# ForJadeForest/DistillCLIP

Hardware: AMD Instinct MI355X
Metric: image-text pairs/sec (distill step) (higher is better)
Workload: dtype bf16; 1 GPU; l_clip.yaml dual distill: ViT-B/32 CLIP teacher -> weight-shared ViT(6x768,24h,R2) + text(4x768,12h,R2) students, 224px/77tok, losses out_l1+out_cos+0.1*cos_diff, fwd+loss+bwd+AdamW; global_batch=512, batch_per_gpu=512, parallelism=dp1, gradient_exchange=none, negatives=local (reference training_step semantics), optimizer_in_step=True, teacher_residual=fp16, saved_gelu_derivative=u8 fixed point, clock_probe=True

## Files before the change

distillclip_amd/csrc/encoder.cpp:

```cpp
#include <math.h>
#include <stdlib.h>
#include <string.h>
#include <new>
#include <vector>
#include "common.h"

namespace {

#define CK(expr)                      \
    do {                              \
        int _rc = (expr);             \
        if (_rc != DCLIP_OK) return _rc; \
    } while (0)

enum { P_PER_TBLOCK = 12, P_PER_SBLOCK = 8, P_PER_SREPEAT = 6 };

struct Plan {
    dclip_encoder_cfg c;
    int D, H, hd, N, Np, F, E, L, R;
    int K;
    int Kp;
    bool student, image, compressed;
    bool mixing;
    bool train;
    struct EmbP { int table, w, bias, cls, pos, ln_w, ln_b; } emb;
    int p_blocks;
    struct HeadP { int norm_w, norm_b, head_w, head_b; } head;
    int n_params;
    struct BlockW { int64_t qkv, qkv_t, proj, proj_t, fc1, fc1_t, fc2, fc2_t; };
    std::vector<BlockW> bw;
    int64_t w_embed, w_embed_t, w_head, w_head_t, w_total;
};

int64_t wtake(int64_t& off, int64_t n) { int64_t o = off; off += (n + 127) & ~(int64_t)127; return o; }

bool make_plan(const dclip_encoder_cfg& c, Plan& p) {
    p.c = c;
    p.student = c.kind == 1; p.train = c.kind != 0; p.image = c.modality == 0; p.mixing = p.student && c.head_mix;
    p.D = c.width; p.H = c.heads; p.N = c.tokens; p.F = c.mlp_dim; p.E = c.out_dim; p.L = c.layers; p.R = c.repeats;
    if (c.kind < 0 || c.kind > 2 || c.modality < 0 || c.modality > 1) { dclip_set_error("encoder: bad kind/modality"); return false; }
    if (p.D <= 0 || p.H <= 0 || p.D % p.H) { dclip_set_error("encoder: width %d not divisible by heads %d", p.D, p.H); return false; }
    p.hd = p.D / p.H;
    if (p.hd != 32 && p.hd != 64) { dclip_set_error("encoder: head dim %d unsupported (32 or 64)", p.hd); return false; }
    if (p.D % 64 || p.F % 64 || p.E % 64 || p.D > 1024) { dclip_set_error("encoder: width/mlp/out dims must be multiples of 64, width <= 1024"); return false; }
    const bool long_ok = c.kind == 0 && p.image && !c.causal && p.hd == 64;
    if (p.N <= 0 || p.N > (long_ok ? 640 : 128)) {
        if (long_ok) dclip_set_error("encoder: tokens must be in 1..640 for a frozen image tower (got %d)", p.N);
        else if (p.N > 128 && c.kind != 0) dclip_set_error("encoder: tokens must be in 1..128 for a trainable tower (kind %d; got %d): only frozen image towers run longer sequences", c.kind, p.N);
        else if (p.N > 128 && !p.image) dclip_set_error("encoder: tokens must be in 1..128 for a text tower (got %d): only frozen image towers run longer sequences", p.N);
        else if (p.N > 128) dclip_set_error("encoder: tokens must be in 1..128 for a causal or head-dim-%d tower (got %d): longer sequences need a non-causal tower with head dim 64", p.hd, p.N);
        else dclip_set_error("encoder: tokens must be in 1..128 (got %d)", p.N);
        return false;
    }
    if (p.L <= 0 || p.R <= 0 || (!p.student && p.R != 1)) { dclip_set_error("encoder: bad layers/repeats"); return false; }
    p.Np = (p.N + 7) & ~7;
    p.compressed = !p.image && c.embed_rank > 0;
    p.K = p.Kp = 0;
    if (p.image) {
        if (c.patch <= 0 || c.resolution < c.patch || c.in_chans <= 0) { dclip_set_error("encoder: bad patch geometry"); return false; }
        const int g = c.resolution / c.patch;
        if (g * g + 1 != p.N) { dclip_set_error("encoder: tokens %d != (res/patch)^2 + 1 = %d", p.N, g * g + 1); return false; }
        p.K = c.in_chans * c.patch * c.patch;
        p.Kp = p.K;
        if (p.K % 64) {
            if (p.train) { dclip_set_error("encoder: in_chans*patch^2 = %d must be a multiple of 64 in a trainable tower", p.K); return false; }
            if (c.patch % 2) { dclip_set_error("encoder: patch %d must be even", c.patch); return false; }
            p.Kp = (p.K + 63) & ~63;
        }
    } else {
        if (c.vocab <= 0) { dclip_set_error("encoder: vocab required for text"); return false; }
        if (p.compressed && c.embed_rank % 64) { dclip_set_error("encoder: embed_rank must be a multiple of 64"); return false; }
        if (p.compressed && !p.student) { dclip_set_error("encoder: a compressed token embedding exists for the weight-shared student only (kind 1)"); return false; }
        if (p.compressed) p.K = p.Kp = c.embed_rank;
    }
    if (p.mixing && p.H != 2 && p.H != 4 && p.H != 8 && p.H != 12 && p.H != 24) {
        dclip_set_error("encoder: head count %d unsupported by the head-mixing kernels", p.H); return false;
    }
    int n = 0;
    Plan::EmbP& em = p.emb;
    em = Plan::EmbP{-1, -1, -1, -1, -1, -1, -1};
    if (p.image) {
        em.w = n++;
        if (p.student) em.bias = n++;
        em.cls = n++; em.pos = n++;
        if (!p.student) { em.ln_w = n++; em.ln_b = n++; }
    } else {
        em.table = n++;
        if (p.compressed) { em.w = n++; em.bias = n++; }
        em.pos = n++;
    }
    p.p_blocks = n;
    n += p.student ? p.L * (P_PER_SBLOCK + p.R * P_PER_SREPEAT) : p.L * P_PER_TBLOCK;
    p.head.norm_w = n++; p.head.norm_b = n++; p.head.head_w = n++;
    p.head.head_b = p.student ? n++ : -1;
    p.n_params = n;
    int64_t off = 0;
    const int64_t D = p.D, F = p.F, E = p.E;
    p.bw.resize(p.L);
    for (int l = 0; l < p.L; ++l) {
        auto& b = p.bw[l];
        b.qkv = wtake(off, 3 * D * D); b.proj = wtake(off, D * D); b.fc1 = wtake(off, F * D); b.fc2 = wtake(off, D * F);
        if (p.train) { b.qkv_t = wtake(off, 3 * D * D); b.proj_t = wtake(off, D * D); b.fc1_t = wtake(off, F * D); b.fc2_t = wtake(off, D * F); }
        else b.qkv_t = b.proj_t = b.fc1_t = b.fc2_t = -1;
    }
    p.w_embed = p.w_embed_t = -1;
    if (em.w >= 0) p.w_embed = wtake(off, D * p.Kp);
    if (p.compressed) p.w_embed_t = wtake(off, D * p.K);
    p.w_head = wtake(off, E * D);
    p.w_head_t = p.train ? wtake(off, E * D) : -1;
    p.w_total = off;
    return true;
}

enum class AttnPath { Fused, Mix, Unfused };
inline AttnPath attn_path(const Plan& p, bool training) {
    static const int mode = [] { const char* e = getenv("DCLIP_ATTN_MIX"); return e ? atoi(e) : 1; }();
    if (!training && !p.mixing) return AttnPath::Fused;
    if (p.mixing && mode != 0 && !p.c.causal && dclip_attn_mix_supported(p.H, p.N, p.hd) != 0) return AttnPath::Mix;
    return AttnPath::Unfused;
}

struct ExecSave {
    void* x_mid;
    float* mean1; float* rstd1; float* mean2; float* rstd2;
    bf16_t *h1, *qkv, *ctx, *h2, *u;
    uint8_t* z;
    float* S;
    bf16_t* P;
    bf16_t* Rm;
    float* stats;
};

void take_scores(Bump& b, const Plan& p, AttnPath path, int64_t B, int64_t N, int64_t Np, ExecSave& s) {
    const int64_t SN = B * p.H * N * Np;
    const bool unfused = path == AttnPath::Unfused;
    s.S = unfused ? b.take<float>(SN) : nullptr;
    s.P = unfused ? b.take<bf16_t>(SN) : nullptr;
    s.Rm = p.mixing ? b.take<bf16_t>(SN) : s.P;
    s.stats = path == AttnPath::Mix ? b.take<float>(B * p.H * N) : nullptr;
}

struct RowSet {
    bf16_t* ctx;
    void *xin, *x_mid, *xout;
    bf16_t *h2, *u;
    float *mean2, *rstd2; uint8_t* z;
    int64_t rows;
};

struct Work {
    std::vector<void*> X;
    bool h16;
    std::vector<ExecSave> ex;
    bf16_t* patches;
    float* tok_table;
    int32_t* pick;
    float *meanf, *rstdf;
    bf16_t* hf;
    void* x0;
    float *mean0, *rstd0;
    float* G0;
    float* G; bf16_t* Gb;
    bf16_t *gb_f2, *gb_pr;
    bf16_t *dbig, *dh, *dqkv, *dout;
    bf16_t* dR;
    bf16_t* dS;
    float* tok_sum; float* demb;
    float* wg_dummy;
    float* mix_ws; size_t mix_ws_bytes;
    void* tn_ws; size_t tn_ws_bytes;
    RowSet compact;
    bf16_t* ctx_full;
    float* Gc;
    AttnPath path;
    size_t bytes;
};

void layout(const Plan& p, int64_t B, bool training, void* base, Work& w, int64_t N = 0) {
    Bump b(base);
    w = Work{};
    if (N <= 0) N = p.N;
    const int64_t Npad = (N + 7) & ~(int64_t)7;
    const int64_t M = B * N, D = p.D, F = p.F, SN = B * p.H * N * Npad;
    const int nex = p.L * p.R;
    const bool save = p.train && training;
    w.path = attn_path(p, save);
    const bool mix = w.path == AttnPath::Mix, unfused = w.path == AttnPath::Unfused;
    w.X.assign(nex + 1, nullptr);
    w.ex.assign(nex, ExecSave{});
    ExecSave shared{};
    void* xs = nullptr;
    w.h16 = !p.train;
    if (!save) {
        xs = w.h16 ? (void*)b.take<_Float16>(M * D) : (void*)b.take<float>(M * D);
        shared.x_mid = xs;
        shared.h1 = b.take<bf16_t>(M * D); shared.qkv = b.take<bf16_t>(M * 3 * D);
        take_scores(b, p, w.path, B, N, Npad, shared);
        shared.ctx = b.take<bf16_t>(M * D); shared.h2 = shared.h1; shared.u = b.take<bf16_t>(M * F);
    }
    for (int e = 0; e <= nex; ++e) w.X[e] = save ? (void*)b.take<float>(M * D) : xs;
    for (int e = 0; e < nex; ++e) {
        if (!save) { w.ex[e] = shared; continue; }
        ExecSave& s = w.ex[e];
        s.x_mid = b.take<float>(M * D);
        s.mean1 = b.take<float>(M); s.rstd1 = b.take<float>(M); s.mean2 = b.take<float>(M); s.rstd2 = b.take<float>(M);
        s.qkv = b.take<bf16_t>(M * 3 * D);
        take_scores(b, p, w.path, B, N, Npad, s);
        s.z = b.take<uint8_t>(M * F);
        if (e % p.R == 0) {
            bf16_t* h1 = b.take<bf16_t>(p.R * M * D); bf16_t* ctx = b.take<bf16_t>(p.R * M * D);
            bf16_t* h2 = b.take<bf16_t>(p.R * M * D); bf16_t* u = b.take<bf16_t>(p.R * M * F);
            for (int r = 0; r < p.R; ++r) {
                ExecSave& t = w.ex[e + r];
                t.h1 = h1 + r * M * D; t.ctx = ctx + r * M * D; t.h2 = h2 + r * M * D; t.u = u + r * M * F;
            }
        }
    }
    {
        const ExecSave& s = w.ex[nex - 1];
        if (save) {
            w.ctx_full = s.h2;
            w.compact = RowSet{s.ctx, w.X[nex], s.x_mid, w.X[nex], s.h2, s.u, s.mean2, s.rstd2, s.z, B};
        } else {
            w.ctx_full = shared.ctx;
            bf16_t* cctx = b.take<bf16_t>(B * D);
            const size_t es = w.h16 ? 2 : 4;
            void* xr = b.take<char>(B * D * es); void* xmc = b.take<char>(B * D * es); void* xoc = b.take<char>(B * D * es);
            w.compact = RowSet{cctx, xr, xmc, xoc, shared.h1, shared.u, nullptr, nullptr, nullptr, B};
        }
        w.Gc = save ? b.take<float>(B * D) : nullptr;
    }
    w.patches = p.emb.w >= 0 ? b.take<bf16_t>(M * p.Kp) : nullptr;
    w.tok_table = b.take<float>((int64_t)N * D);
    w.pick = b.take<int32_t>(B);
    w.meanf = b.take<float>(B); w.rstdf = b.take<float>(B);
    w.hf = b.take<bf16_t>(B * D);
    const bool pre_ln = p.emb.ln_w >= 0, pre = save && pre_ln;
    w.x0 = pre_ln ? (w.h16 ? (void*)b.take<_Float16>(M * D) : (void*)b.take<float>(M * D)) : nullptr;
    w.mean0 = pre ? b.take<float>(M) : nullptr; w.rstd0 = pre ? b.take<float>(M) : nullptr; w.G0 = pre ? b.take<float>(M * D) : nullptr;
    if (save) {
        w.G = b.take<float>(M * D); w.Gb = b.take<bf16_t>(M * D);
        w.gb_f2 = b.take<bf16_t>(p.R * M * D); w.gb_pr = b.take<bf16_t>(p.R * M * D);
        w.dbig = b.take<bf16_t>(p.R * M * F); w.dh = b.take<bf16_t>(M * D); w.dqkv = b.take<bf16_t>(p.R * M * 3 * D);
        w.dR = unfused ? b.take<bf16_t>(SN) : nullptr; w.dS = b.take<bf16_t>(SN); w.dout = b.take<bf16_t>(B * p.E);
        w.tok_sum = b.take<float>((int64_t)N * D);
        w.wg_dummy = mix ? b.take<float>(2 * p.H * p.H) : nullptr;
        w.mix_ws_bytes = mix ? dclip_attn_mix_bwd_workspace_bytes(B, p.H, N) : 0;
        w.mix_ws = w.mix_ws_bytes ? (float*)b.take<char>(w.mix_ws_bytes) : nullptr;
        w.tn_ws_bytes = dclip_gemm_tn_workspace_bytes();
        w.tn_ws = b.take<char>(w.tn_ws_bytes);
        w.demb = p.compressed ? b.take<float>(M * p.K) : nullptr;
    }
    w.bytes = b.off;
}

inline RowSet full_rows(const Work& w, int ei, int64_t M) {
    const ExecSave& s = w.ex[ei];
    return RowSet{s.ctx, w.X[ei], s.x_mid, w.X[ei + 1], s.h2, s.u, s.mean2, s.rstd2, s.z, M};
}

inline const float* PF(const void* const* params, int i) { return i < 0 ? nullptr : (const float*)params[i]; }

inline int wsplits(int64_t M, int64_t P, int64_t Q) {
    const double tiles = (double)((P + 127) / 128) * (double)((Q + 127) / 128);
    const int smax = (int)((M + 255) / 256);
    int best = 1;
    double best_t = 1e30;
    for (int s = 1; s <= smax && s <= 64; ++s) {
        const double blocks = tiles * s;
        const double rounds = ceil(blocks / 512.0);
        const double t_mm = rounds * (2.0 * 128 * 128 * ((double)M / s)) / 1.76e12;
        const double t_at = 0.5 * s * (double)P * Q * 4.0 / 1.3e12;
        const double t = t_mm + t_at + 2e-6;
        if (t < best_t) { best_t = t; best = s; }
    }
    return best;
}

inline int gemm(const void* A, int64_t lda, const void* Bw, int64_t ldb, void* C, int64_t ldc, int64_t M, int64_t N, int64_t K,
                const float* bias, int act, const void* aux_in, void* aux_out, const void* res, int64_t ldr, int out_dtype,
                int64_t row_group, const float* rowadd, void* st) {
    return dclip_gemm_nt(A, lda, Bw, ldb, C, ldc, M, N, K, 1.f, bias, act, aux_in, aux_out, res, ldr, out_dtype, row_group, rowadd, nullptr, st);
}

inline int ln_stream(bool h16, const void* x, int64_t ldx, const int32_t* ridx, const float* g, const float* b, void* y, int64_t ldy, int out_dtype,
                     float* mean, float* rstd, int64_t M, int64_t D, void* st) {
    if (h16) return dclip_layernorm_fwd_f16(x, ldx, ridx, g, b, y, ldy, out_dtype, mean, rstd, M, D, 1e-5f, st);
    return dclip_layernorm_fwd((const float*)x, ldx, ridx, g, b, y, ldy, out_dtype, mean, rstd, M, D, 1e-5f, st);
}

inline int export_stream(bool h16, const void* src, float* dst, int64_t n, void* st) {
    if (h16) return dclip_cast_f16_f32(src, dst, n, st);
    if (hipMemcpyAsync(dst, src, (size_t)n * 4, hipMemcpyDeviceToDevice, (hipStream_t)st) != hipSuccess) {
        dclip_set_error("dclip_encoder_forward: hidden-state export failed");
        return DCLIP_ELAUNCH;
    }
    return DCLIP_OK;
}

int attn_forward(AttnPath path, const Plan& p, const ExecSave& s, const float* wl, const float* ww, int64_t B, int64_t N, const int32_t* pick,
                 void* st) {
    const int64_t D = p.D, H = p.H, hd = p.hd, Np = (N + 7) & ~(int64_t)7;
    const float scale = 1.f / sqrtf((float)hd);
    if (path == AttnPath::Fused) {
        if (N <= 128 && pick) return dclip_attn_fused_fwd_rows(s.qkv, 3 * D, s.ctx, D, B, H, N, hd, scale, p.c.causal, pick, st);
        if (N <= 128) return dclip_attn_fused_fwd(s.qkv, 3 * D, s.ctx, D, B, H, N, hd, scale, p.c.causal, st);
        return dclip_attn_stream_fwd(s.qkv, 3 * D, s.ctx, D, B, H, N, hd, scale, st);
    }
    const int blk = path == AttnPath::Mix ? 1 : 0;
    if (path == AttnPath::Mix) {
        if (pick) CK(dclip_attn_mix_fwd_rows(s.qkv, 3 * D, wl, ww, s.Rm, s.stats, B, H, N, Np, hd, scale, pick, st));
        else CK(dclip_attn_mix_fwd(s.qkv, 3 * D, wl, ww, s.Rm, s.stats, B, H, N, Np, hd, scale, st));
    } else {
        CK(dclip_attn_nt(s.qkv, 3 * D, s.qkv + D, 3 * D, s.S, 1, B, H, N, Np, hd, scale, st));
        CK(dclip_attn_softmax_fwd(s.S, wl, ww, wl ? s.P : nullptr, s.Rm, B, H, N, Np, p.c.causal, st));
    }
    if (pick) return dclip_attn_nn_rows(s.Rm, s.qkv + 2 * D, 3 * D, s.ctx, D, B, H, N, Np, hd, 1.f, blk, pick, 0, st);
    return dclip_attn_nn(s.Rm, s.qkv + 2 * D, 3 * D, s.ctx, D, B, H, N, Np, hd, 1.f, blk, st);
}

struct MapGrad { const float* d_score; const float* d_prob; void* scratch; size_t scratch_bytes; };
int attn_backward(AttnPath path, const Plan& p, const ExecSave& s, const Work& w, const float* wl, const float* ww, float* gl, float* gw,
                  const bf16_t* dctx, bf16_t* dqkv, int64_t B, const MapGrad* mg, const int32_t* pick, void* st) {
    const int64_t D = p.D, H = p.H, hd = p.hd, N = p.N, Np = p.Np;
    const float scale = 1.f / sqrtf((float)hd);
    const int blk = path == AttnPath::Mix ? 1 : 0;
    if (pick) {
        CK(dclip_attn_tn_rows(s.Rm, dctx, D, dqkv + 2 * D, 3 * D, B, H, N, Np, hd, 1.f, blk, pick, st));
        if (path == AttnPath::Mix) {
            CK(dclip_attn_mix_bwd_rows(s.qkv, 3 * D, dctx, D, wl, ww, s.stats, w.dS, gl ? gl : w.wg_dummy, gw ? gw : w.wg_dummy + H * H,
                                       w.mix_ws, w.mix_ws_bytes, B, H, N, Np, hd, scale, pick, st));
        } else {
            CK(dclip_attn_nt(dctx, D, s.qkv + 2 * D, 3 * D, w.dR, 0, B, H, N, Np, hd, 1.f, st));
            CK(dclip_attn_softmax_bwd(w.dR, s.P, s.S, 0, wl, ww, w.dS, gl, gw, B, H, N, Np, st));
        }
        CK(dclip_attn_nn_rows(w.dS, s.qkv + D, 3 * D, dqkv, 3 * D, B, H, N, Np, hd, scale, blk, pick, 1, st));
        return dclip_attn_tn_rows(w.dS, s.qkv, 3 * D, dqkv + D, 3 * D, B, H, N, Np, hd, scale, blk, pick, st);
    }
    CK(dclip_attn_tn(s.Rm, dctx, D, dqkv + 2 * D, 3 * D, B, H, N, Np, hd, 1.f, blk, st));
    if (path == AttnPath::Mix) {
        CK(dclip_attn_mix_bwd(s.qkv, 3 * D, dctx, D, wl, ww, s.stats, w.dS, gl ? gl : w.wg_dummy, gw ? gw : w.wg_dummy + H * H,
                              w.mix_ws, w.mix_ws_bytes, B, H, N, Np, hd, scale, st));
    } else {
        CK(dclip_attn_nt(dctx, D, s.qkv + 2 * D, 3 * D, w.dR, 0, B, H, N, Np, hd, 1.f, st));
        CK(dclip_attn_softmax_bwd(w.dR, s.P, s.S, 0, wl, ww, w.dS, gl, gw, B, H, N, Np, st));
    }
    if (mg) CK(dclip_attn_maps_bwd(s.qkv, 3 * D, wl, mg->d_score, mg->d_prob, w.dS, blk, gl, mg->scratch, mg->scratch_bytes, B, H, N, Np, hd,
                                   scale, p.c.causal, st));
    CK(dclip_attn_nn(w.dS, s.qkv + D, 3 * D, dqkv, 3 * D, B, H, N, Np, hd, scale, blk, st));
    return dclip_attn_tn(w.dS, s.qkv, 3 * D, dqkv + D, 3 * D, B, H, N, Np, hd, scale, blk, st);
}

}

enum : uint32_t { RUN_SEEDS_CLEAR = 1u, RUN_PRUNED = 2u, RUN_PRUNED_ATTN = 4u };

struct dclip_encoder { Plan p; };

extern "C" dclip_encoder* dclip_encoder_create(const dclip_encoder_cfg* cfg) {
    if (!cfg) { dclip_set_error("dclip_encoder_create: null cfg"); return nullptr; }
    dclip_encoder* e = new (std::nothrow) dclip_encoder();
    if (!e) { dclip_set_error("dclip_encoder_create: out of host memory"); return nullptr; }
    if (!make_plan(*cfg, e->p)) { delete e; return nullptr; }
    return e;
}

extern "C" void dclip_encoder_destroy(dclip_encoder* e) { delete e; }
extern "C" int64_t dclip_encoder_num_params(const dclip_encoder* e) { return e ? e->p.n_params : -1; }
extern "C" size_t dclip_encoder_wcache_bytes(const dclip_encoder* e) { return e ? dclip_up256((size_t)e->p.w_total * 2) : 0; }

extern "C" size_t dclip_encoder_workspace_bytes(const dclip_encoder* e, int64_t B, int training) {
    if (!e || B <= 0) return 0;
    Work w;
    layout(e->p, B, training != 0, nullptr, w);
    return w.bytes;
}

namespace {
struct BX { int n1w, n1b, n2w, n2b, qkvw, qkvb, prw, prb, f1w, f1b, f2w, f2b, cl, cw; };
inline BX bexec(const Plan& p, int l, int r) {
    if (!p.student) {
        const int b = p.p_blocks + l * P_PER_TBLOCK;
        return BX{b, b + 1, b + 6, b + 7, b + 2, b + 3, b + 4, b + 5, b + 8, b + 9, b + 10, b + 11, -1, -1};
    }
    const int b = p.p_blocks + l * (P_PER_SBLOCK + p.R * P_PER_SREPEAT), q = b + P_PER_SBLOCK + r * P_PER_SREPEAT;
    return BX{q, q + 1, q + 2, q + 3, b, b + 1, b + 2, b + 3, b + 4, b + 5, b + 6, b + 7, q + 4, q + 5};
}

struct EP { const float *n1w, *n1b, *n2w, *n2b, *bq, *bp, *b1, *b2, *wl, *ww; };
inline EP exec_params(const Plan& p, const void* const* params, int l, int r) {
    const BX bx = bexec(p, l, r);
    EP e{PF(params, bx.n1w), PF(params, bx.n1b), PF(params, bx.n2w), PF(params, bx.n2b), PF(params, bx.qkvb), PF(params, bx.prb),
         PF(params, bx.f1b), PF(params, bx.f2b), nullptr, nullptr};
    if (p.mixing) { e.wl = PF(params, bx.cl); e.ww = PF(params, bx.cw); }
    return e;
}

int exec_attn(const Plan& p, AttnPath path, const ExecSave& s, const bf16_t* W, int l, const EP& e, bool h16, const void* xin, int64_t B,
              int64_t N, const int32_t* pick, void* st) {
    const int64_t D = p.D, M = B * N;
    CK(ln_stream(h16, xin, D, nullptr, e.n1w, e.n1b, s.h1, D, DCLIP_OUT_BF16, s.mean1, s.rstd1, M, D, st));
    CK(gemm(s.h1, D, W + p.bw[l].qkv, D, s.qkv, 3 * D, M, 3 * D, D, e.bq, 0, nullptr, nullptr, nullptr, 0, DCLIP_OUT_BF16, 0, nullptr, st));
    return attn_forward(path, p, s, e.wl, e.ww, B, N, pick, st);
}

int exec_mlp(const Plan& p, const bf16_t* W, int l, const EP& e, bool h16, const RowSet& rs, void* st) {
    const int64_t D = p.D, F = p.F, rows = rs.rows;
    const auto& bw = p.bw[l];
    const int sdt = h16 ? DCLIP_OUT_F16 : DCLIP_OUT_F32;
    const int act = p.student ? (rs.z ? DCLIP_ACT_GELU_SAVE : DCLIP_ACT_GELU) : (rs.z ? DCLIP_ACT_QUICKGELU_SAVE : DCLIP_ACT_QUICKGELU);
    CK(gemm(rs.ctx, D, W + bw.proj, D, rs.x_mid, D, rows, D, D, e.bp, 0, nullptr, nullptr, rs.xin, D, sdt, 0, nullptr, st));
    CK(ln_stream(h16, rs.x_mid, D, nullptr, e.n2w, e.n2b, rs.h2, D, DCLIP_OUT_BF16, rs.mean2, rs.rstd2, rows, D, st));
    CK(gemm(rs.h2, D, W + bw.fc1, D, rs.u, F, rows, F, D, e.b1, act, nullptr, rs.z, nullptr, 0, DCLIP_OUT_BF16, 0, nullptr, st));
    return gemm(rs.u, F, W + bw.fc2, F, rs.xout, D, rows, D, F, e.b2, 0, nullptr, nullptr, rs.x_mid, D, sdt, 0, nullptr, st);
}

size_t llo_scratch(const Plan& p, AttnPath path, bool h16, int64_t B, void* base, void* xin, ExecSave& t, RowSet& rs) {
    Bump b(base);
    const int64_t N = p.N, M = B * N, D = p.D, F = p.F;
    const size_t es = h16 ? 2 : 4;
    t = ExecSave{};
    t.h1 = b.take<bf16_t>(M * D); t.h2 = t.h1;
    t.qkv = b.take<bf16_t>(M * 3 * D);
    take_scores(b, p, path, B, N, p.Np, t);
    t.ctx = b.take<bf16_t>(M * D);
    t.x_mid = b.take<char>(M * D * es);
    t.u = b.take<bf16_t>(M * F);
    rs = RowSet{t.ctx, xin, t.x_mid, b.take<char>(M * D * es), t.h2, t.u, nullptr, nullptr, nullptr, M};
    return b.off;
}

inline bool prune_last_enabled() {
    static const int v = [] { const char* e = getenv("DCLIP_PRUNE_LAST"); return e ? atoi(e) : 1; }();
    return v != 0;
}
inline bool prune_attn_enabled() {
    static const int v = [] { const char* e = getenv("DCLIP_PRUNE_ATTN"); return e ? atoi(e) : 1; }();
    return v != 0;
}

template <class T> struct ExecMaps { std::vector<T*> score, prob; uint64_t score_bits = 0, prob_bits = 0; };
template <class T>
int exec_maps(const Plan& p, const dclip_attn_maps* maps, T* const* score, T* const* prob, const dclip_encoder_run* rec, const char* fn,
              ExecMaps<T>& out) {
    const int nex = p.L * p.R;
    out.score.assign(nex, nullptr); out.prob.assign(nex, nullptr);
    if (!maps || !maps->n) return DCLIP_OK;
    DCLIP_REQUIRE(maps->n > 0 && maps->exec, "%s: maps need n > 0 execution indices", fn);
    for (int k = 0; k < maps->n; ++k) {
        const int ei = maps->exec[k];
        DCLIP_REQUIRE(ei >= 0 && ei < nex, "%s: map %d: block execution %d out of range 0..%d", fn, k, ei, nex - 1);
        T* sm = score ? score[k] : nullptr;
        T* pm = prob ? prob[k] : nullptr;
        if (!rec) {
            DCLIP_REQUIRE(ei < 64, "%s: map %d: block execution %d: maps are exported for executions 0..63 only", fn, k, ei);
        } else {
            const bool had_s = ei < 64 && (rec->score_maps >> ei & 1), had_p = ei < 64 && (rec->prob_maps >> ei & 1);
            DCLIP_REQUIRE((!sm || had_s) && (!pm || had_p), "%s: a gradient for the %s map of block execution %d, which the forward did not export",
                          fn, sm && !had_s ? "score" : "probability", ei);
        }
        if (sm) { out.score[ei] = sm; out.score_bits |= (uint64_t)1 << ei; }
        if (pm) { out.prob[ei] = pm; out.prob_bits |= (uint64_t)1 << ei; }
    }
    return DCLIP_OK;
}
}

extern "C" int dclip_encoder_prepare(const dclip_encoder* e, const void* const* params, void* wcache, void* st) {
    DCLIP_REQUIRE(e && params && wcache, "dclip_encoder_prepare: null argument");
    const Plan& p = e->p;
    bf16_t* W = (bf16_t*)wcache;
    const int64_t D = p.D, F = p.F, E = p.E;
    auto at = [&](int64_t off) -> void* { return off < 0 ? nullptr : (void*)(W + off); };
    std::vector<const float*> src; std::vector<void*> wb, wt; std::vector<int64_t> rr, cc;
    auto job = [&](const float* w, void* b, void* t, int64_t R, int64_t C) { src.push_back(w); wb.push_back(b); wt.push_back(t); rr.push_back(R); cc.push_back(C); };
    for (int l = 0; l < p.L; ++l) {
        const auto& b = p.bw[l];
        const BX bx = bexec(p, l, 0);
        job(PF(params, bx.qkvw), at(b.qkv), at(b.qkv_t), 3 * D, D);
        job(PF(params, bx.prw), at(b.proj), at(b.proj_t), D, D);
        job(PF(params, bx.f1w), at(b.fc1), at(b.fc1_t), F, D);
        job(PF(params, bx.f2w), at(b.fc2), at(b.fc2_t), D, F);
    }
    const bool pad_embed = p.Kp != p.K;
    if (p.emb.w >= 0 && !pad_embed) job(PF(params, p.emb.w), at(p.w_embed), at(p.w_embed_t), D, p.K);
    if (p.student) job(PF(params, p.head.head_w), at(p.w_head), at(p.w_head_t), E, D);
    else job(PF(params, p.head.head_w), at(p.w_head_t), at(p.w_head), D, E);
    for (size_t i = 0; i < src.size(); ++i) DCLIP_REQUIRE(src[i], "dclip_encoder_prepare: parameter %zu missing", i);
    if (pad_embed) {
        DCLIP_REQUIRE(PF(params, p.emb.w), "dclip_encoder_prepare: the patch-embedding weight is missing");
        CK(dclip_cast_bf16_pad(PF(params, p.emb.w), at(p.w_embed), D, p.K, p.Kp, st));
    }
    return dclip_cast_transpose_bf16_multi(src.data(), wb.data(), wt.data(), rr.data(), cc.data(), (int64_t)src.size(), st);
}

static int clear_backward_seeds(const Plan& p, const Work& w, int64_t M, int64_t B, bool pruned, void* st) {
    const int64_t D = p.D;
    hipStream_t hs = (hipStream_t)st;
    bf16_t* gb_last = w.gb_f2 + (int64_t)(p.R - 1) * M * D;
    const bool ok = pruned ? hipMemsetAsync(w.Gc, 0, (size_t)B * D * 4, hs) == hipSuccess
                           : hipMemsetAsync(w.G, 0, (size_t)M * D * 4, hs) == hipSuccess && hipMemsetAsync(gb_last, 0, (size_t)M * D * 2, hs) == hipSuccess;
    if (!ok) { dclip_set_error("dclip_encoder: clearing the backward seeds failed"); return DCLIP_ELAUNCH; }
    return DCLIP_OK;
}

extern "C" int dclip_encoder_forward(const dclip_encoder* e, const void* input, const void* patches, int64_t B, const void* const* params,
                                     const void* wcache, void* workspace, size_t ws_bytes, dclip_encoder_run* run, int training,
                                     float* last_representation, float* const* rep_out, float* emb_out, int64_t tokens_eff,
                                     const dclip_attn_maps* maps, void* st) {
    DCLIP_REQUIRE(e && (input || patches) && params && wcache && workspace && run && last_representation, "dclip_encoder_forward: null argument");
    DCLIP_REQUIRE(B > 0, "dclip_encoder_forward: empty batch");
    const Plan& p = e->p;
    const bf16_t* ext_patches = (const bf16_t*)patches;
    DCLIP_REQUIRE(!ext_patches || (p.image && ((uintptr_t)ext_patches % 16) == 0), "dclip_encoder_forward: patches: image towers only, 16-byte aligned rows");
    DCLIP_REQUIRE(!ext_patches || tokens_eff == 0, "dclip_encoder_forward: patches cannot be combined with tokens_eff");
    DCLIP_REQUIRE(!ext_patches || p.Kp == p.K, "dclip_encoder_forward: this tower pads its patch rows (%d -> %d columns) and cuts them itself: pass the images", p.K, p.Kp);
    DCLIP_REQUIRE(!training || p.train, "dclip_encoder_forward: the frozen teacher tower (kind 0) is inference-only");
    DCLIP_REQUIRE(tokens_eff == 0 || (!p.train && !p.image && p.c.causal && tokens_eff > 0 && tokens_eff <= p.N && !rep_out && !emb_out),
                  "dclip_encoder_forward: tokens_eff is only valid for the causal text teacher without hidden-state export");
    DCLIP_REQUIRE(!(maps && maps->n > 0 && maps->exec) || tokens_eff == 0,
                  "dclip_encoder_forward: attention maps cannot be exported from a caption prefix (tokens_eff)");
    DCLIP_REQUIRE(!(maps && maps->n > 0) || p.N <= 128,
                  "dclip_encoder_forward: attention maps cannot be exported from a tower of %d tokens (dclip_attn_maps_fwd / _bwd take N <= 128)", p.N);
    ExecMaps<float> xm;
    CK(exec_maps<float>(p, maps, maps ? maps->score : nullptr, maps ? maps->prob : nullptr, nullptr, "dclip_encoder_forward", xm));
    Work w;
    layout(p, B, training != 0, workspace, w, tokens_eff);
    DCLIP_REQUIRE(ws_bytes >= w.bytes, "dclip_encoder_forward: workspace too small (%zu < %zu)", ws_bytes, w.bytes);
    DCLIP_REQUIRE(((uintptr_t)workspace % 256) == 0 && ((uintptr_t)wcache % 256) == 0, "dclip_encoder_forward: buffers must be 256-byte aligned");
    const bf16_t* W = (const bf16_t*)wcache;
    const int64_t N = tokens_eff ? tokens_eff : p.N, D = p.D, F = p.F, E = p.E, M = B * N;
    const int nex = p.L * p.R;

    const Plan::EmbP& em = p.emb;
    const bool pre_ln = em.ln_w >= 0;
    const int sdt = w.h16 ? DCLIP_OUT_F16 : DCLIP_OUT_F32;
    if (em.w >= 0) {
        const bf16_t* rows = ext_patches ? ext_patches : w.patches;
        if (!p.image) CK(dclip_embed_gather((const int64_t*)input, p.N, PF(params, em.table), nullptr, w.patches, 0, M, N, p.K, st));
        else if (!ext_patches && p.Kp != p.K) CK(dclip_im2row_ld((const float*)input, w.patches, p.Kp, B, p.c.in_chans, p.c.resolution, p.c.patch, 1, st));
        else if (!ext_patches) CK(dclip_im2row((const float*)input, w.patches, B, p.c.in_chans, p.c.resolution, p.c.patch, 1, st));
        CK(dclip_token_table(PF(params, em.pos), PF(params, em.cls), PF(params, em.bias), w.tok_table, N, D, st));
        CK(gemm(rows, p.Kp, W + p.w_embed, p.Kp, pre_ln ? w.x0 : w.X[0], D, M, D, p.Kp, nullptr, 0, nullptr, nullptr, nullptr, 0, sdt, N, w.tok_table, st));
        if (pre_ln) CK(ln_stream(w.h16, w.x0, D, nullptr, PF(params, em.ln_w), PF(params, em.ln_b), w.X[0], D, sdt, w.mean0, w.rstd0, M, D, st));
    } else {
        CK(dclip_embed_gather((const int64_t*)input, p.N, PF(params, em.table), PF(params, em.pos), w.X[0], sdt, M, N, D, st));
    }

    if (emb_out) CK(export_stream(w.h16, pre_ln ? w.x0 : w.X[0], emb_out, M * D, st));

    CK(dclip_pick_index(p.image ? nullptr : (const int64_t*)input, p.N, w.pick, B, N, st));
    const bool prune = prune_last_enabled() && !(rep_out && rep_out[nex - 1]) && !xm.score[nex - 1] && !xm.prob[nex - 1];
    const bool prune_attn = prune && prune_attn_enabled() && N <= 128;
    for (int ei = 0; ei < nex; ++ei) {
        const int l = ei / p.R, r = ei % p.R;
        const ExecSave& s = w.ex[ei];
        const EP ep = exec_params(p, params, l, r);
        const bool compact = prune && ei == nex - 1;
        ExecSave sa = s;
        if (compact) sa.ctx = w.ctx_full;
        CK(exec_attn(p, w.path, sa, W, l, ep, w.h16, w.X[ei], B, N, compact && prune_attn ? w.pick : nullptr, st));
        if (xm.score[ei] || xm.prob[ei]) CK(dclip_attn_maps_fwd(s.qkv, 3 * D, ep.wl, xm.score[ei], xm.prob[ei], B, p.H, N, p.hd, 1.f / sqrtf((float)p.hd), p.c.causal, st));
        if (compact) {
            CK(dclip_rows_pick(w.ctx_full, w.compact.ctx, w.pick, B, D * 2, st));
            CK(dclip_rows_pick(w.X[ei], w.compact.xin, w.pick, B, D * (w.h16 ? 2 : 4), st));
        }
        CK(exec_mlp(p, W, l, ep, w.h16, compact ? w.compact : full_rows(w, ei, M), st));
        if (rep_out && rep_out[ei]) CK(export_stream(w.h16, w.X[ei + 1], rep_out[ei], M * D, st));
    }

    CK(ln_stream(w.h16, prune ? w.compact.xout : w.X[nex], D, prune ? nullptr : w.pick, PF(params, p.head.norm_w), PF(params, p.head.norm_b), w.hf, D,
                 DCLIP_OUT_BF16, w.meanf, w.rstdf, B, D, st));
    CK(gemm(w.hf, D, W + p.w_head, D, last_representation, E, B, E, D, PF(params, p.head.head_b), 0, nullptr, nullptr, nullptr, 0, DCLIP_OUT_F32, 0, nullptr, st));
    *run = dclip_encoder_run{(prune ? RUN_PRUNED : 0u) | (prune_attn ? RUN_PRUNED_ATTN : 0u), 0, 0, 0};
    if (training) {
        CK(clear_backward_seeds(p, w, M, B, prune, st));
        run->flags |= RUN_SEEDS_CLEAR;
        run->score_maps = xm.score_bits;
        run->prob_maps = xm.prob_bits;
    }
    return DCLIP_OK;
}

extern "C" size_t dclip_encoder_last_layer_output_scratch_bytes(const dclip_encoder* e, int64_t B, int training) {
    if (!e || B <= 0) return 0;
    const Plan& p = e->p;
    ExecSave t;
    RowSet rs;
    return llo_scratch(p, attn_path(p, p.train && training != 0), !p.train, B, nullptr, nullptr, t, rs);
}

extern "C" int dclip_encoder_last_layer_output(const dclip_encoder* e, int64_t B, const void* const* params, const void* wcache,
                                               void* workspace, size_t ws_bytes, const dclip_encoder_run* run, int training, void* scratch,
                                               float* out, void* st) {
    DCLIP_REQUIRE(e && params && wcache && workspace && run && scratch && out, "dclip_encoder_last_layer_output: null argument");
    DCLIP_REQUIRE(B > 0, "dclip_encoder_last_layer_output: empty batch");
    const Plan& p = e->p;
    DCLIP_REQUIRE(!training || p.train, "dclip_encoder_last_layer_output: the frozen teacher tower (kind 0) is inference-only");
    Work w;
    layout(p, B, training != 0, workspace, w);
    DCLIP_REQUIRE(ws_bytes >= w.bytes, "dclip_encoder_last_layer_output: workspace too small (%zu < %zu)", ws_bytes, w.bytes);
    const bf16_t* W = (const bf16_t*)wcache;
    const int64_t M = B * p.N, D = p.D, E = p.E;
    const int nex = p.L * p.R;
    const void* xlast = w.X[nex];
    if (run->flags & RUN_PRUNED) {
        ExecSave t;
        RowSet rs;
        const int ei = nex - 1, l = ei / p.R;
        llo_scratch(p, w.path, w.h16, B, scratch, w.X[ei], t, rs);
        const EP ep = exec_params(p, params, l, ei % p.R);
        CK(exec_attn(p, w.path, t, W, l, ep, w.h16, w.X[ei], B, p.N, nullptr, st));
        CK(exec_mlp(p, W, l, ep, w.h16, rs, st));
        xlast = rs.xout;
    }
    CK(ln_stream(w.h16, xlast, D, nullptr, PF(params, p.head.norm_w), PF(params, p.head.norm_b), scratch, D, DCLIP_OUT_BF16, nullptr, nullptr, M, D, st));
    CK(gemm(scratch, D, W + p.w_head, D, out, E, M, E, D, PF(params, p.head.head_b), 0, nullptr, nullptr, nullptr, 0, DCLIP_OUT_F32, 0, nullptr, st));
    return DCLIP_OK;
}

extern "C" int dclip_encoder_backward(const dclip_encoder* e, const void* input, const void* patches, int64_t B, const void* const* params,
                                      void* const* grads, const void* wcache, void* workspace, size_t ws_bytes, dclip_encoder_run* run,
                                      const float* d_last_representation, const float* const* d_rep, const float* d_emb,
                                      const dclip_attn_maps* maps, dclip_bucket_cb on_bucket, void* cb_user, void* st) {
    DCLIP_REQUIRE(e && (input || patches) && params && grads && wcache && workspace && run && d_last_representation, "dclip_encoder_backward: null argument");
    const Plan& p = e->p;
    const bf16_t* ext_patches = (const bf16_t*)patches;
    DCLIP_REQUIRE(!ext_patches || p.image, "dclip_encoder_backward: patches: image towers only");
    DCLIP_REQUIRE(p.train, "dclip_encoder_backward: the frozen teacher tower (kind 0) has no backward");
    ExecMaps<const float> gm;
    CK(exec_maps<const float>(p, maps, maps ? maps->d_score : nullptr, maps ? maps->d_prob : nullptr, run, "dclip_encoder_backward", gm));
    if (p.mixing && gm.prob_bits) {
        const size_t need = dclip_attn_maps_bwd_workspace_bytes(B, p.H, p.N);
        DCLIP_REQUIRE(maps->scratch && maps->scratch_bytes >= need,
                      "dclip_encoder_backward: probability-map gradients of a head-mixing tower need %zu bytes of maps scratch", need);
    }
    Work w;
    layout(p, B, true, workspace, w);
    DCLIP_REQUIRE(ws_bytes >= w.bytes, "dclip_encoder_backward: workspace too small");
    const bf16_t* W = (const bf16_t*)wcache;
    const int64_t N = p.N, D = p.D, F = p.F, E = p.E, M = B * N;
    const int nex = p.L * p.R;
    const bool pruned = (run->flags & RUN_PRUNED) != 0;
    DCLIP_REQUIRE(!pruned || !(d_rep && d_rep[nex - 1]),
                  "dclip_encoder_backward: a gradient for the hidden state of block execution %d, which the forward ran on the class / EOT "
                  "rows only (request that hidden state in the forward, or set DCLIP_PRUNE_LAST=0)", nex - 1);
    DCLIP_REQUIRE(!pruned || !(gm.score[nex - 1] || gm.prob[nex - 1]),
                  "dclip_encoder_backward: a map gradient for block execution %d, which the forward ran on the class / EOT rows only", nex - 1);
    auto GR = [&](int i) -> float* { return i < 0 ? nullptr : (float*)grads[i]; };
    hipStream_t hs = (hipStream_t)st;

    if (run->flags & RUN_SEEDS_CLEAR) run->flags &= ~RUN_SEEDS_CLEAR;
    else CK(clear_backward_seeds(p, w, M, B, pruned, st));
    CK(dclip_cast_bf16(d_last_representation, w.dout, B * E, st));
    if (p.student) {
        if (GR(p.head.head_w)) CK(dclip_gemm_tn_acc(w.dout, E, w.hf, D, GR(p.head.head_w), D, B, E, D, 1, w.tn_ws, w.tn_ws_bytes, st));
        if (GR(p.head.head_b)) CK(dclip_colsum_acc(w.dout, E, GR(p.head.head_b), B, E, st));
    } else if (GR(p.head.head_w)) {
        CK(dclip_gemm_tn_acc(w.hf, D, w.dout, E, GR(p.head.head_w), E, B, D, E, 1, w.tn_ws, w.tn_ws_bytes, st));
    }
    CK(gemm(w.dout, E, W + p.w_head_t, E, w.dh, D, B, D, E, nullptr, 0, nullptr, nullptr, nullptr, 0, DCLIP_OUT_BF16, 0, nullptr, st));
    const int R = p.R;
    bf16_t* gb_last = w.gb_f2 + (int64_t)(R - 1) * M * D;
    CK(dclip_layernorm_bwd(w.dh, D, 0, (const float*)(pruned ? w.compact.xout : w.X[nex]), D, pruned ? nullptr : w.pick, PF(params, p.head.norm_w), w.meanf,
                           w.rstdf, pruned ? w.Gc : w.G, D, gb_last, D, GR(p.head.norm_w), GR(p.head.norm_b), GR(bexec(p, (nex - 1) / p.R, 0).f2b), B, D, st));
    if (on_bucket) on_bucket(cb_user, 0);

    for (int ei = nex - 1; ei >= 0; --ei) {
        const int l = ei / p.R, r = ei % p.R;
        const auto& bw = p.bw[l];
        const ExecSave& s = w.ex[ei];
        const BX bx = bexec(p, l, r);
        const float *wl = nullptr, *ww = nullptr;
        float *gl = nullptr, *gw = nullptr;
        if (p.mixing) { wl = PF(params, bx.cl); ww = PF(params, bx.cw); gl = GR(bx.cl); gw = GR(bx.cw); }
        bf16_t* gb_f2 = w.gb_f2 + (int64_t)r * M * D;
        bf16_t* gb_pr = w.gb_pr + (int64_t)r * M * D;
        bf16_t* dbig = w.dbig + (int64_t)r * M * F;
        bf16_t* dqkv = w.dqkv + (int64_t)r * M * 3 * D;
        const int64_t MR = (int64_t)R * M;
        const ExecSave& s0 = w.ex[ei - r];
        const bool compact = pruned && ei == nex - 1;
        const RowSet rs = compact ? w.compact : full_rows(w, ei, M);
        const int64_t Mx = rs.rows;
        const int64_t MRw = pruned && l == p.L - 1 ? (int64_t)(R - 1) * M + B : MR;
        if (d_rep && d_rep[ei]) CK(dclip_axpy_f32(w.G, d_rep[ei], gb_f2, M * D, GR(bx.f2b), D, st));
        CK(dclip_gemm_nt(gb_f2, D, W + bw.fc2_t, D, dbig, F, Mx, F, D, 1.f, nullptr, DCLIP_ACT_MULAUX, rs.z, nullptr, nullptr, 0, DCLIP_OUT_BF16, 0, nullptr,
                         GR(bx.f1b), st));
        if (r == 0 && GR(bx.f2w)) CK(dclip_gemm_tn_acc(w.gb_f2, D, s0.u, F, GR(bx.f2w), F, MRw, D, F, wsplits(MRw, D, F), w.tn_ws, w.tn_ws_bytes, st));
        if (r == 0 && GR(bx.f1w)) CK(dclip_gemm_tn_acc(w.dbig, F, s0.h2, D, GR(bx.f1w), D, MRw, F, D, wsplits(MRw, F, D), w.tn_ws, w.tn_ws_bytes, st));
        CK(gemm(dbig, F, W + bw.fc1_t, F, w.dh, D, Mx, D, F, nullptr, 0, nullptr, nullptr, nullptr, 0, DCLIP_OUT_BF16, 0, nullptr, st));
        CK(dclip_layernorm_bwd(w.dh, D, 0, (const float*)rs.x_mid, D, nullptr, PF(params, bx.n2w), rs.mean2, rs.rstd2, compact ? w.Gc : w.G, D, gb_pr, D,
                               GR(bx.n2w), GR(bx.n2b), GR(bx.prb), Mx, D, st));
        if (r == 0 && GR(bx.prw)) CK(dclip_gemm_tn_acc(w.gb_pr, D, s0.ctx, D, GR(bx.prw), D, MRw, D, D, wsplits(MRw, D, D), w.tn_ws, w.tn_ws_bytes, st));
        bf16_t* dctx = w.dh;
        if (!compact) {
            CK(gemm(gb_pr, D, W + bw.proj_t, D, dctx, D, M, D, D, nullptr, 0, nullptr, nullptr, nullptr, 0, DCLIP_OUT_BF16, 0, nullptr, st));
        } else {
            bf16_t* dctx_c = dqkv;
            CK(gemm(gb_pr, D, W + bw.proj_t, D, dctx_c, D, B, D, D, nullptr, 0, nullptr, nullptr, nullptr, 0, DCLIP_OUT_BF16, 0, nullptr, st));
            CK(dclip_rows_expand(dctx_c, dctx, w.pick, B, N, D * 2, st));
            CK(dclip_rows_expand(w.Gc, w.G, w.pick, B, N, D * 4, st));
        }
        const MapGrad mg{gm.score[ei], gm.prob[ei], maps ? maps->scratch : nullptr, maps ? maps->scratch_bytes : 0};
        CK(attn_backward(w.path, p, s, w, wl, ww, gl, gw, dctx, dqkv, B, mg.d_score || mg.d_prob ? &mg : nullptr,
                         compact && (run->flags & RUN_PRUNED_ATTN) ? w.pick : nullptr, st));
        if (r == 0 && GR(bx.qkvw)) CK(dclip_gemm_tn_acc(w.dqkv, 3 * D, s0.h1, D, GR(bx.qkvw), D, MR, 3 * D, D, wsplits(MR, 3 * D, D), w.tn_ws, w.tn_ws_bytes, st));
        if (r == 0 && params[bx.qkvb] && GR(bx.qkvb)) CK(dclip_colsum_acc(w.dqkv, 3 * D, GR(bx.qkvb), MR, 3 * D, st));
        CK(gemm(dqkv, 3 * D, W + bw.qkv_t, 3 * D, w.dh, D, M, D, 3 * D, nullptr, 0, nullptr, nullptr, nullptr, 0, DCLIP_OUT_BF16, 0, nullptr, st));
        bf16_t* gb_next = ei > 0 ? w.gb_f2 + (int64_t)((ei - 1) % R) * M * D : w.Gb;
        CK(dclip_layernorm_bwd(w.dh, D, 0, (const float*)w.X[ei], D, nullptr, PF(params, bx.n1w), s.mean1, s.rstd1, w.G, D, gb_next, D, GR(bx.n1w), GR(bx.n1b),
                               ei > 0 ? GR(bexec(p, (ei - 1) / p.R, 0).f2b) : nullptr, M, D, st));
        if (r == 0 && on_bucket) on_bucket(cb_user, 1 + (p.L - 1 - l));
    }

    const Plan::EmbP& em = p.emb;
    const bool pre_ln = em.ln_w >= 0;
    if (d_emb && !pre_ln) CK(dclip_axpy_f32(w.G, d_emb, w.Gb, M * D, nullptr, D, st));
    if (hipMemsetAsync(w.tok_sum, 0, (size_t)N * D * 4, hs) != hipSuccess) { dclip_set_error("dclip_encoder_backward: memset failed"); return DCLIP_ELAUNCH; }
    const float* Ge = w.G;
    if (pre_ln) {
        if (hipMemsetAsync(w.G0, 0, (size_t)M * D * 4, hs) != hipSuccess) { dclip_set_error("dclip_encoder_backward: memset failed"); return DCLIP_ELAUNCH; }
        CK(dclip_layernorm_bwd(w.G, D, 1, (const float*)w.x0, D, nullptr, PF(params, em.ln_w), w.mean0, w.rstd0, w.G0, D, w.Gb, D, GR(em.ln_w), GR(em.ln_b),
                               nullptr, M, D, st));
        if (d_emb) CK(dclip_axpy_f32(w.G0, d_emb, w.Gb, M * D, nullptr, D, st));
        Ge = w.G0;
    }
    if (em.w >= 0) {
        const int64_t K = p.K;
        const bf16_t* rows = ext_patches ? ext_patches : w.patches;
        if (GR(em.w)) CK(dclip_gemm_tn_acc(w.Gb, D, rows, K, GR(em.w), K, M, D, K, wsplits(M, D, K), w.tn_ws, w.tn_ws_bytes, st));
        if (GR(em.bias) || GR(em.cls) || GR(em.pos)) {
            CK(dclip_batch_sum_acc(Ge, w.tok_sum, B, N, D, st));
            CK(dclip_token_table_bwd(w.tok_sum, GR(em.pos), GR(em.cls), GR(em.bias), N, D, p.image ? 1 : 0, st));
        }
        if (GR(em.table)) {
            CK(gemm(w.Gb, D, W + p.w_embed_t, D, w.demb, K, M, K, D, nullptr, 0, nullptr, nullptr, nullptr, 0, DCLIP_OUT_F32, 0, nullptr, st));
            CK(dclip_embed_scatter_add((const int64_t*)input, w.demb, 1, GR(em.table), M, K, p.c.vocab, st));
        }
    } else {
        if (GR(em.table)) CK(dclip_embed_scatter_add((const int64_t*)input, w.G, 1, GR(em.table), M, D, p.c.vocab, st));
        if (GR(em.pos)) {
            CK(dclip_batch_sum_acc(w.G, w.tok_sum, B, N, D, st));
            CK(dclip_token_table_bwd(w.tok_sum, GR(em.pos), nullptr, nullptr, N, D, 0, st));
        }
    }
    if (on_bucket) on_bucket(cb_user, p.L + 1);
    return DCLIP_OK;
}

extern "C" int32_t dclip_encoder_num_grad_buckets(const dclip_encoder* e) { return e ? e->p.L + 2 : -1; }
extern "C" int dclip_encoder_grad_bucket(const dclip_encoder* e, int32_t bucket, int32_t* first_param, int32_t* end_param) {
    DCLIP_REQUIRE(e && first_param && end_param, "dclip_encoder_grad_bucket: null argument");
    const Plan& p = e->p;
    DCLIP_REQUIRE(bucket >= 0 && bucket <= p.L + 1, "dclip_encoder_grad_bucket: bucket %d out of range 0..%d", bucket, p.L + 1);
    const int per_block = p.student ? P_PER_SBLOCK + p.R * P_PER_SREPEAT : P_PER_TBLOCK;
    if (bucket == 0) { *first_param = p.head.norm_w; *end_param = p.n_params; }
    else if (bucket == p.L + 1) { *first_param = 0; *end_param = p.p_blocks; }
    else { const int l = p.L - bucket; *first_param = p.p_blocks + l * per_block; *end_param = *first_param + per_block; }
    return DCLIP_OK;
}
```

distillclip_amd/csrc/gemm_tn.hip:

```cpp

#include "gemm_common.h"
#include <atomic>

using namespace dgemm;

namespace {

constexpr int TP = 128, TQ = 128, TC = 64;
constexpr int TROW = 288;
constexpr int TTILE = TC * TROW;

struct GemmTN {
    const bf16_t* A; int64_t lda;
    const bf16_t* B; int64_t ldb;
    float* out; int64_t ldo;
    int M, P, Q;
    int tiles_p, tiles_q, splits, chunk;
    unsigned long long* stamps;
    float* partial;
};

__device__ __forceinline__ void tn_load(const bf16_t* __restrict__ G, int64_t ld, int m0, int m_end, int c0, int cols,
                                        int tid, u32x4 (&regs)[4]) {
#pragma unroll
    for (int s = 0; s < 4; ++s) {
        const int idx = s * 256 + tid;
        const int r = idx >> 4, c = (idx & 15) * 8;
        const int row = m0 + r, col = c0 + c;
        if (row < m_end && col < cols) regs[s] = *(const u32x4*)(G + (int64_t)row * ld + col);
        else regs[s] = u32x4{0u, 0u, 0u, 0u};
    }
}
__device__ __forceinline__ void tn_store(char* tile, int tid, const u32x4 (&regs)[4]) {
#pragma unroll
    for (int s = 0; s < 4; ++s) {
        const int idx = s * 256 + tid;
        const int r = idx >> 4, c = (idx & 15);
        *(u32x4*)(tile + r * TROW + c * 16) = regs[s];
    }
}

__global__ __launch_bounds__(256) void gemm_tn_kernel(GemmTN p) {
    extern __shared__ __attribute__((aligned(16))) char smem[];
    const int tid = threadIdx.x, lane = tid & 63;
    const int wave = __builtin_amdgcn_readfirstlane(tid >> 6);
    const int wp = wave >> 1, wq = wave & 1;

    int t = blockIdx.x;
    const int split = t % p.splits; t /= p.splits;
    const int tq = t % p.tiles_q, tp = t / p.tiles_q;
    const int p0 = tp * TP, q0 = tq * TQ;
    const int m_begin = split * p.chunk;
    const int m_end = min(p.M, m_begin + p.chunk);
    if (m_begin >= m_end) return;

    char* As = smem;
    char* Bs = smem + 2 * TTILE;

    f32x4 acc[4][4];
#pragma unroll
    for (int i = 0; i < 4; ++i)
#pragma unroll
        for (int j = 0; j < 4; ++j) acc[i][j] = f32x4{0.f, 0.f, 0.f, 0.f};

    u32x4 ra[4], rb[4];
    const int nc = (m_end - m_begin + TC - 1) / TC;
    tn_load(p.A, p.lda, m_begin, m_end, p0, p.P, tid, ra);
    tn_load(p.B, p.ldb, m_begin, m_end, q0, p.Q, tid, rb);
    tn_store(As, tid, ra);
    tn_store(Bs, tid, rb);

    for (int ct = 0; ct < nc; ++ct) {
        __syncthreads();
        const bool more = ct + 1 < nc;
        if (more) {
            tn_load(p.A, p.lda, m_begin + (ct + 1) * TC, m_end, p0, p.P, tid, ra);
            tn_load(p.B, p.ldb, m_begin + (ct + 1) * TC, m_end, q0, p.Q, tid, rb);
        }
        const char* a_t = As + (ct & 1) * TTILE;
        const char* b_t = Bs + (ct & 1) * TTILE;
#pragma unroll
        for (int kb = 0; kb < 2; ++kb) {
            bf16x8 af[4], bfr[4];
#pragma unroll
            for (int i = 0; i < 4; ++i) af[i] = tr_frag<TROW>(a_t, kb * 32, wp * 64 + i * 16, lane);
#pragma unroll
            for (int j = 0; j < 4; ++j) bfr[j] = tr_frag<TROW>(b_t, kb * 32, wq * 64 + j * 16, lane);
            mfma_4x4(acc, af, bfr);
        }
        if (more) {
            tn_store(As + ((ct + 1) & 1) * TTILE, tid, ra);
            tn_store(Bs + ((ct + 1) & 1) * TTILE, tid, rb);
        }
    }

    const int colb = q0 + wq * 64 + (lane & 15);
    const int rowb = p0 + wp * 64 + (lane >> 4) * 4;
#pragma unroll
    for (int i = 0; i < 4; ++i)
#pragma unroll
        for (int r = 0; r < 4; ++r) {
            const int row = rowb + i * 16 + r;
            if (row >= p.P) continue;
#pragma unroll
            for (int j = 0; j < 4; ++j) {
                const int col = colb + j * 16;
                if (col < p.Q) unsafeAtomicAdd(p.out + (int64_t)row * p.ldo + col, acc[i][j][r]);
            }
        }
}

constexpr int TNB = TC * 256;
constexpr int TCLD = 128 + 4;
constexpr int TN_LDS = (4 * TNB > 128 * TCLD * 4) ? 4 * TNB : 128 * TCLD * 4;

__device__ __forceinline__ int tn_key(int row) { return 2 * ((row & 3) | (((row >> 3) & 1) << 2)); }

struct TnWork { int split, tile, p0, q0, m_begin, m_end; };
template <int EDGE>
__device__ __forceinline__ TnWork tn_locate(const GemmTN& p) {
    const int tiles = p.tiles_p * p.tiles_q;
    const int t = xcd_remap(blockIdx.x, tiles * p.splits);
    TnWork w;
    w.split = t / tiles; w.tile = t - w.split * tiles;
    const int tq = w.tile % p.tiles_q, tp = w.tile / p.tiles_q;
    w.p0 = tp * EDGE; w.q0 = tq * EDGE;
    w.m_begin = w.split * p.chunk;
    w.m_end = min(p.M, w.m_begin + p.chunk);
    return w;
}

template <int NP, bool CLAMP>
__device__ __forceinline__ void tn_sources(const bf16_t* __restrict__ G, int64_t ld, int m0, int c0, int cols, int wave, int lane,
                                           const char* (&src)[NP]) {
#pragma unroll
    for (int s = 0; s < NP; ++s) {
        const int piece = wave * NP + s;
        const int r = piece * 4 + (lane >> 4);
        const int lc = (lane & 15) ^ tn_key(r);
        const bf16_t* rowp = G + (int64_t)(m0 + r) * ld;
        const int col = c0 + lc * 8;
        src[s] = (const char*)(CLAMP ? rowp + (col < cols ? col : cols - 8) : rowp + c0 + lc * 8);
    }
}
template <int NP>
__device__ __forceinline__ void tn_stage(const char* const (&src)[NP], int64_t chunk_off, char* tile, int wave) {
#pragma unroll
    for (int s = 0; s < NP; ++s)
        __builtin_amdgcn_global_load_lds((gbl_void*)(src[s] + chunk_off), (lds_void*)(tile + (wave * NP + s) * 1024), 16, 0, 0);
}

template <int OFF>
__device__ __forceinline__ bf16x8 tr_frag_asm(unsigned base) {
    s16x4 lo, hi;
    asm volatile("ds_read_b64_tr_b16 %0, %1 offset:%2" : "=v"(lo) : "v"(base), "n"(OFF));
    asm volatile("ds_read_b64_tr_b16 %0, %1 offset:%2" : "=v"(hi) : "v"(base), "n"(OFF + 4 * 256));
    return frag_halves(lo, hi);
}
__device__ __forceinline__ unsigned tr_frag_base(const char* tile, int x0, int lane) {
    const int g = lane >> 4, q = (lane >> 2) & 3, pp = lane & 3;
    const int row = 8 * g + q;
    const int chunk = (x0 >> 3) + (pp >> 1);
    return (unsigned)(uintptr_t)(tile + row * 256 + ((chunk ^ tn_key(row)) << 4) + (pp & 1) * 8);
}

__global__ __launch_bounds__(256) void gemm_tn_glds_kernel(GemmTN p) {
    extern __shared__ __attribute__((aligned(16))) char smem[];
    const int tid = threadIdx.x, lane = tid & 63;
    const int wave = __builtin_amdgcn_readfirstlane(tid >> 6);
    const int wp = wave >> 1, wq = wave & 1;

    const TnWork w = tn_locate<TP>(p);
    const int p0 = w.p0, q0 = w.q0, m_begin = w.m_begin, m_end = w.m_end;
    if (m_begin >= m_end) return;
    const int nc = (m_end - m_begin) / TC;

    char* As = smem;
    char* Bs = smem + 2 * TNB;
    f32x4 acc[4][4];
#pragma unroll
    for (int i = 0; i < 4; ++i)
#pragma unroll
        for (int j = 0; j < 4; ++j) acc[i][j] = f32x4{0.f, 0.f, 0.f, 0.f};

    const char* src_a[4];
    const char* src_b[4];
    tn_sources<4, true>(p.A, p.lda, m_begin, p0, p.P, wave, lane, src_a);
    tn_sources<4, true>(p.B, p.ldb, m_begin, q0, p.Q, wave, lane, src_b);
    const int64_t step_a = (int64_t)TC * p.lda * 2, step_b = (int64_t)TC * p.ldb * 2;
    tn_stage(src_a, 0, As, wave);
    tn_stage(src_b, 0, Bs, wave);
    for (int ct = 0; ct < nc; ++ct) {
        __syncthreads();
        if (ct + 1 < nc) {
            const int nb = (ct + 1) & 1;
            tn_stage(src_a, (ct + 1) * step_a, As + nb * TNB, wave);
            tn_stage(src_b, (ct + 1) * step_b, Bs + nb * TNB, wave);
        }
        const char* a_t = As + (ct & 1) * TNB;
        const char* b_t = Bs + (ct & 1) * TNB;
        unsigned abase[4], bbase[4];
#pragma unroll
        for (int i = 0; i < 4; ++i) { abase[i] = tr_frag_base(a_t, wp * 64 + i * 16, lane); bbase[i] = tr_frag_base(b_t, wq * 64 + i * 16, lane); }
        bf16x8 af[2][4], bfr[2][4];
#pragma unroll
        for (int i = 0; i < 4; ++i) { af[0][i] = tr_frag_asm<0>(abase[i]); bfr[0][i] = tr_frag_asm<0>(bbase[i]); }
#pragma unroll
        for (int i = 0; i < 4; ++i) { af[1][i] = tr_frag_asm<32 * 256>(abase[i]); bfr[1][i] = tr_frag_asm<32 * 256>(bbase[i]); }
        WAIT_LGKM0();
        __builtin_amdgcn_sched_barrier(0);
#pragma unroll
        for (int kb = 0; kb < 2; ++kb) mfma_4x4(acc, af[kb], bfr[kb]);
    }
    __syncthreads();
    float* cs = (float*)smem;
    stage_acc<4, TCLD>(cs, acc, wp * 64, wq * 64, lane);
    __syncthreads();
#pragma unroll 4
    for (int it = 0; it < 64; ++it) {
        const int rl = wave * 32 + (it >> 1), cl = (it & 1) * 64 + lane;
        const int row = p0 + rl, col = q0 + cl;
        if (row < p.P && col < p.Q) unsafeAtomicAdd(p.out + (int64_t)row * p.ldo + col, cs[rl * TCLD + cl]);
    }
}

__global__ __launch_bounds__(512) void gemm_tn256_kernel(GemmTN p) {
    extern __shared__ __attribute__((aligned(16))) char smem[];
    const int tid = threadIdx.x, lane = tid & 63;
    const int wave = __builtin_amdgcn_readfirstlane(tid >> 6);
    const int wr = wave >> 2, wc = wave & 3;

    const TnWork w = tn_locate<256>(p);
    const int p0 = w.p0, q0 = w.q0, m_begin = w.m_begin, m_end = w.m_end;
    if (m_begin >= m_end) return;
    const int nk = (m_end - m_begin) / TC;
    const int nload = 4 * nk;

    f32x4 acc[8][4];
#pragma unroll
    for (int i = 0; i < 8; ++i)
#pragma unroll
        for (int j = 0; j < 4; ++j) acc[i][j] = f32x4{0.f, 0.f, 0.f, 0.f};

    const char* srcs[4][2];
    tn_sources<2, false>(p.B, p.ldb, m_begin, q0, p.Q, wave, lane, srcs[0]);
    tn_sources<2, false>(p.B, p.ldb, m_begin, q0 + 128, p.Q, wave, lane, srcs[1]);
    tn_sources<2, false>(p.A, p.lda, m_begin, p0, p.P, wave, lane, srcs[2]);
    tn_sources<2, false>(p.A, p.lda, m_begin, p0 + 128, p.P, wave, lane, srcs[3]);
    const int64_t step_b = (int64_t)TC * p.ldb * 2, step_a = (int64_t)TC * p.lda * 2;
    auto issue = [&](int l) {
        const int kt = l >> 2, hw = l & 3;
        char* buf = smem + ((kt & 1) * 4 + hw) * HT;
        if (hw == 0) tn_stage(srcs[0], kt * step_b, buf, wave);
        else if (hw == 1) tn_stage(srcs[1], kt * step_b, buf, wave);
        else if (hw == 2) tn_stage(srcs[2], kt * step_a, buf, wave);
        else tn_stage(srcs[3], kt * step_a, buf, wave);
    };
    wg_stamp(p.stamps, tid, 0);
    const int npro = nload < 6 ? nload : 6;
#pragma unroll
    for (int l = 0; l < 6; ++l)
        if (l < npro) issue(l);
    if (nload > 4) WAIT_VMCNT(4); else WAIT_VMCNT(0);
    __builtin_amdgcn_s_barrier();
    wg_stamp(p.stamps, tid, 1);
    if (wr == 1) __builtin_amdgcn_s_barrier();

    const int a_off = (2 + wr) * HT;
    const int b_off = (wc >> 1) * HT;
    const int bcol = (wc & 1) * 64;
    bf16x8 af[4][2], b0[2][2], b1[2][2];

    for (int kt = 0; kt < nk; ++kt) {
        const char* base = smem + (kt & 1) * 4 * HT;
        const char* at = base + a_off;
        const char* bt = base + b_off;
        const int k4 = kt * 4;
#pragma unroll
        for (int j = 0; j < 2; ++j) {
            const unsigned a0 = tr_frag_base(bt, bcol + j * 16, lane), a1 = tr_frag_base(bt, bcol + (2 + j) * 16, lane);
            b0[j][0] = tr_frag_asm<0>(a0); b0[j][1] = tr_frag_asm<32 * 256>(a0);
            b1[j][0] = tr_frag_asm<0>(a1); b1[j][1] = tr_frag_asm<32 * 256>(a1);
        }
        __builtin_amdgcn_sched_barrier(0);
#pragma unroll
        for (int i = 0; i < 4; ++i) {
            const unsigned a0 = tr_frag_base(at, i * 16, lane);
            af[i][0] = tr_frag_asm<0>(a0); af[i][1] = tr_frag_asm<32 * 256>(a0);
        }
        if (k4 + 6 < nload) issue(k4 + 6);
        if (k4 + 7 < nload) issue(k4 + 7);
        WAIT_LGKM0();
        __builtin_amdgcn_sched_barrier(0);
        PHASE_MFMA(false, acc, 0, 4, af, b0, b1);
        __builtin_amdgcn_sched_barrier(0);
#pragma unroll
        for (int i = 0; i < 4; ++i) {
            const unsigned a0 = tr_frag_base(at, (4 + i) * 16, lane);
            af[i][0] = tr_frag_asm<0>(a0); af[i][1] = tr_frag_asm<32 * 256>(a0);
        }
        if (k4 + 8 < nload) { issue(k4 + 8); issue(k4 + 9); WAIT_VMCNT(4); }
        else WAIT_VMCNT(0);
        WAIT_LGKM0();
        __builtin_amdgcn_sched_barrier(0);
        PHASE_MFMA(false, acc, 4, 4, af, b0, b1);
    }
    if (wr == 0) __builtin_amdgcn_s_barrier();
    wg_stamp(p.stamps, tid, 2);

    float* cs = (float*)smem;
    constexpr int CL = 256 + 4;
#pragma unroll
    for (int q = 0; q < 4; ++q) {
        __syncthreads();
        stage_acc<2, CL>(cs, acc + q * 2, wr * 32, wc * 64, lane);
        __syncthreads();
        if (p.partial) {
            float* dst = p.partial + ((int64_t)w.split * (p.tiles_p * p.tiles_q) + w.tile) * 65536;
#pragma unroll 4
            for (int it = 0; it < 8; ++it) {
                const int sl = (tid >> 6) + it * 8;
                const int rt = (sl >> 5) * 128 + q * 32 + (sl & 31);
                *(float4*)(dst + rt * 256 + (tid & 63) * 4) = *(const float4*)&cs[sl * CL + (tid & 63) * 4];
            }
        } else {
#pragma unroll 4
            for (int it = 0; it < 32; ++it) {
                const int sl = (tid >> 8) + it * 2;
                const int row = p0 + (sl >> 5) * 128 + q * 32 + (sl & 31);
                const int col = q0 + (tid & 255);
                unsafeAtomicAdd(p.out + (int64_t)row * p.ldo + col, cs[sl * CL + (tid & 255)]);
            }
        }
    }
    wg_stamp(p.stamps, tid, 3);
}

__global__ __launch_bounds__(256) void tn256_reduce_kernel(const float* __restrict__ partial, int splits, int tiles, int tiles_q,
                                                           float* __restrict__ out, int64_t ldo) {
    const int idx = blockIdx.x * 256 + threadIdx.x;
    const int tile = idx >> 14, rt = (idx >> 6) & 255, c4 = idx & 63;
    if (tile >= tiles) return;
    const float* src = partial + (int64_t)tile * 65536 + rt * 256 + c4 * 4;
    float4 a = *(const float4*)src;
    for (int s = 1; s < splits; ++s) {
        const float4 v = *(const float4*)(src + (int64_t)s * tiles * 65536);
        a.x += v.x; a.y += v.y; a.z += v.z; a.w += v.w;
    }
    float* o = out + (int64_t)((tile / tiles_q) * 256 + rt) * ldo + (tile % tiles_q) * 256 + c4 * 4;
    float4 cur = *(const float4*)o;
    cur.x += a.x; cur.y += a.y; cur.z += a.z; cur.w += a.w;
    *(float4*)o = cur;
}

__global__ __launch_bounds__(256) void colsum_kernel(const bf16_t* __restrict__ X, int64_t ld, float* __restrict__ db,
                                                     int M, int N, int rows_per_block) {
    const int col = blockIdx.x * 256 + threadIdx.x;
    if (col >= N) return;
    const int r0 = blockIdx.y * rows_per_block;
    const int r1 = min(M, r0 + rows_per_block);
    float s0 = 0.f, s1 = 0.f, s2 = 0.f, s3 = 0.f;
    int r = r0;
    for (; r + 3 < r1; r += 4) {
        s0 += bf2f(X[(int64_t)r * ld + col]);
        s1 += bf2f(X[(int64_t)(r + 1) * ld + col]);
        s2 += bf2f(X[(int64_t)(r + 2) * ld + col]);
        s3 += bf2f(X[(int64_t)(r + 3) * ld + col]);
    }
    for (; r < r1; ++r) s0 += bf2f(X[(int64_t)r * ld + col]);
    unsafeAtomicAdd(db + col, (s0 + s1) + (s2 + s3));
}

__global__ __launch_bounds__(256) void colsum8_kernel(const bf16_t* __restrict__ X, int64_t ld, float* __restrict__ db,
                                                      int M, int N, int rows_per_block) {
    __shared__ float red[8][256 + 8];
    const int cg = threadIdx.x & 31, rl = threadIdx.x >> 5;
    const int col = blockIdx.x * 256 + cg * 8;
    const int r0 = blockIdx.y * rows_per_block;
    const int r1 = min(M, r0 + rows_per_block);
    float acc[8];
#pragma unroll
    for (int e = 0; e < 8; ++e) acc[e] = 0.f;
    if (col < N) {
        int r = r0 + rl;
        for (; r + 24 < r1; r += 32) {
            bf16x8 v[4];
#pragma unroll
            for (int u = 0; u < 4; ++u) v[u] = *(const bf16x8*)(X + (int64_t)(r + 8 * u) * ld + col);
#pragma unroll
            for (int u = 0; u < 4; ++u)
#pragma unroll
                for (int e = 0; e < 8; ++e) acc[e] += bf2f(v[u][e]);
        }
        for (; r < r1; r += 8) {
            const bf16x8 v = *(const bf16x8*)(X + (int64_t)r * ld + col);
#pragma unroll
            for (int e = 0; e < 8; ++e) acc[e] += bf2f(v[e]);
        }
    }
#pragma unroll
    for (int e = 0; e < 8; ++e) red[rl][cg * 8 + e] = acc[e];
    __syncthreads();
    const int c = blockIdx.x * 256 + threadIdx.x;
    if (c < N) {
        float x = 0.f;
#pragma unroll
        for (int w = 0; w < 8; ++w) x += red[w][threadIdx.x];
        unsafeAtomicAdd(db + c, x);
    }
}

std::atomic<long long> g_tn_atomic_fallbacks{0};

void set_splits(GemmTN& p, int splits) {
    const int chunk = (int)(((int64_t)p.M + splits - 1) / splits);
    p.chunk = ((chunk + TC - 1) / TC) * TC;
    p.splits = (p.M + p.chunk - 1) / p.chunk;
}

}

extern "C" int64_t dclip_gemm_tn_atomic_fallbacks(void) { return (int64_t)g_tn_atomic_fallbacks.load(std::memory_order_relaxed); }

extern "C" size_t dclip_gemm_tn_workspace_bytes(void) { return (size_t)384 * 65536 * sizeof(float); }

extern "C" int dclip_gemm_tn_acc(const void* A, int64_t lda, const void* B, int64_t ldb, float* dW, int64_t ldo,
                                 int64_t M, int64_t P, int64_t Q, int splits, void* workspace, size_t ws_bytes, void* stream) {
    DCLIP_REQUIRE(A && B && dW, "dclip_gemm_tn_acc: null operand");
    DCLIP_REQUIRE(M > 0 && P > 0 && Q > 0, "dclip_gemm_tn_acc: empty problem");
    DCLIP_REQUIRE(P % 8 == 0 && Q % 8 == 0 && lda % 8 == 0 && ldb % 8 == 0 &&
                  ((uintptr_t)A % 16) == 0 && ((uintptr_t)B % 16) == 0,
                  "dclip_gemm_tn_acc: P, Q, lda, ldb must be multiples of 8 and bases 16-byte aligned");
    DCLIP_REQUIRE(splits >= 1, "dclip_gemm_tn_acc: splits must be >= 1");
    GemmTN p;
    p.A = (const bf16_t*)A; p.lda = lda; p.B = (const bf16_t*)B; p.ldb = ldb; p.out = dW; p.ldo = ldo;
    p.M = (int)M; p.P = (int)P; p.Q = (int)Q; p.stamps = g_gemm_stamps; p.partial = nullptr;
    const bool fast = M % TC == 0 && P >= 8 && Q >= 8;
    const bool big = fast && P % 256 == 0 && Q % 256 == 0 && (P / 256) * (Q / 256) >= 16 && M >= 4096;
    TraceScope tr(DCLIP_TRACE_GEMM_TN, 2.0 * (double)M * (double)P * (double)Q, 2.0 * ((double)M * P + (double)M * Q) + 4.0 * (double)P * Q, stream, (int)M, (int)P, (int)Q, big ? 256 : 128);
    if (big) {
        p.tiles_p = (int)(P / 256); p.tiles_q = (int)(Q / 256);
        const int tiles = p.tiles_p * p.tiles_q;
        const int s = (256 + tiles / 2) / tiles;
        set_splits(p, s < 1 ? 1 : s);
        static const int tn_partial = [] { const char* e = getenv("DCLIP_TN_PARTIAL"); return e ? atoi(e) : 1; }();
        const size_t need = (size_t)tiles * p.splits * 65536 * sizeof(float);
        const bool part = tn_partial != 0 && workspace && ws_bytes >= need && ldo % 4 == 0 && ((uintptr_t)dW % 16) == 0 && p.splits > 1;
        if (!part && p.splits > 1) g_tn_atomic_fallbacks.fetch_add(1, std::memory_order_relaxed);
        p.partial = part ? (float*)workspace : nullptr;
        hipLaunchKernelGGL(gemm_tn256_kernel, dim3(tiles * p.splits), dim3(512), 8 * HT, (hipStream_t)stream, p);
        if (part)
            hipLaunchKernelGGL(tn256_reduce_kernel, dim3((unsigned)(tiles * 64)), dim3(256), 0, (hipStream_t)stream, (const float*)workspace,
                               p.splits, tiles, p.tiles_q, dW, ldo);
        return dclip_check_launch("dclip_gemm_tn_acc");
    }
    p.tiles_p = (int)((P + TP - 1) / TP); p.tiles_q = (int)((Q + TQ - 1) / TQ);
    set_splits(p, splits);
    const int grid = p.tiles_p * p.tiles_q * p.splits;
    if (fast) hipLaunchKernelGGL(gemm_tn_glds_kernel, dim3(grid), dim3(256), TN_LDS, (hipStream_t)stream, p);
    else hipLaunchKernelGGL(gemm_tn_kernel, dim3(grid), dim3(256), 4 * TTILE, (hipStream_t)stream, p);
    return dclip_check_launch("dclip_gemm_tn_acc");
}

extern "C" int dclip_colsum_acc(const void* X, int64_t ld, float* db, int64_t M, int64_t N, void* stream) {
    DCLIP_REQUIRE(X && db && M > 0 && N > 0, "dclip_colsum_acc: bad argument");
    const int colblocks = (int)((N + 255) / 256);
    int rows_per_block = (int)((M * colblocks + 511) / 512);
    rows_per_block = rows_per_block < 16 ? 16 : (rows_per_block > 512 ? 512 : (rows_per_block + 3) & ~3);
    dim3 grid((unsigned)((N + 255) / 256), (unsigned)((M + rows_per_block - 1) / rows_per_block));
    if (N % 8 == 0 && ld % 8 == 0 && ((uintptr_t)X & 15) == 0)
        hipLaunchKernelGGL(colsum8_kernel, grid, dim3(256), 0, (hipStream_t)stream, (const bf16_t*)X, ld, db, (int)M, (int)N,
                           rows_per_block);
    else
        hipLaunchKernelGGL(colsum_kernel, grid, dim3(256), 0, (hipStream_t)stream, (const bf16_t*)X, ld, db, (int)M, (int)N,
                           rows_per_block);
    return dclip_check_launch("dclip_colsum_acc");
}
```

distillclip_amd/csrc/layernorm.hip:

```cpp
#include <stdlib.h>
#include "common.h"

namespace {

constexpr int LN_MAXV = 4;

template <int NV, int OUT, bool X_F16>
__global__ __launch_bounds__(256) void ln_fwd_kernel(const void* __restrict__ x, int64_t ldx, const int* __restrict__ ridx,
                                                     const float* __restrict__ gamma, const float* __restrict__ beta,
                                                     void* __restrict__ y, int64_t ldy, float* __restrict__ mean,
                                                     float* __restrict__ rstd, int M, int D, float eps) {
    const int lane = threadIdx.x & 63;
    const int row = blockIdx.x * 4 + (threadIdx.x >> 6);
    if (row >= M) return;
    const int64_t src = ridx ? ridx[row] : row;
    float4 v[NV];
    float s = 0.f;
#pragma unroll
    for (int i = 0; i < NV; ++i) {
        const int c = (i * 64 + lane) * 4;
        v[i] = float4{0.f, 0.f, 0.f, 0.f};
        if (c < D) {
            if (X_F16) {
                const f16x4 h = *(const f16x4*)((const _Float16*)x + src * ldx + c);
                v[i] = float4{(float)h[0], (float)h[1], (float)h[2], (float)h[3]};
            } else {
                v[i] = *(const float4*)((const float*)x + src * ldx + c);
            }
        }
        s += (v[i].x + v[i].y) + (v[i].z + v[i].w);
    }
    const float mu = wave_sum(s) / D;
    float q = 0.f;
#pragma unroll
    for (int i = 0; i < NV; ++i) {
        const int c = (i * 64 + lane) * 4;
        if (c < D) {
            const float a = v[i].x - mu, b = v[i].y - mu, cc = v[i].z - mu, d = v[i].w - mu;
            q += (a * a + b * b) + (cc * cc + d * d);
        }
    }
    const float rs = rsqrtf(wave_sum(q) / D + eps);
    if (lane == 0) {
        if (mean) mean[row] = mu;
        if (rstd) rstd[row] = rs;
    }
#pragma unroll
    for (int i = 0; i < NV; ++i) {
        const int c = (i * 64 + lane) * 4;
        if (c < D) {
            const float4 g = *(const float4*)(gamma + c), b = *(const float4*)(beta + c);
            const float o0 = (v[i].x - mu) * rs * g.x + b.x, o1 = (v[i].y - mu) * rs * g.y + b.y;
            const float o2 = (v[i].z - mu) * rs * g.z + b.z, o3 = (v[i].w - mu) * rs * g.w + b.w;
            if (OUT == 1) {
                *(float4*)((float*)y + (int64_t)row * ldy + c) = float4{o0, o1, o2, o3};
            } else if (OUT == 2) {
                *(f16x4*)((_Float16*)y + (int64_t)row * ldy + c) = f16x4{(_Float16)o0, (_Float16)o1, (_Float16)o2, (_Float16)o3};
            } else {
                bf16x4 o = {f2bf(o0), f2bf(o1), f2bf(o2), f2bf(o3)};
                *(bf16x4*)((bf16_t*)y + (int64_t)row * ldy + c) = o;
            }
        }
    }
}

template <int NV, bool DY_F32>
__global__ __launch_bounds__(512) void ln_bwd_kernel(const void* __restrict__ dy, int64_t lddy, const float* __restrict__ x,
                                                     int64_t ldx, const int* __restrict__ ridx,
                                                     const float* __restrict__ gamma, const float* __restrict__ mean,
                                                     const float* __restrict__ rstd, float* __restrict__ dx_acc,
                                                     int64_t lddx, bf16_t* __restrict__ dx_bf16, int64_t lddb,
                                                     float* __restrict__ dgamma, float* __restrict__ dbeta, float* __restrict__ colsum, int M, int D) {
    constexpr int NW = 8, DP = NV * 256;
    extern __shared__ float red_[];
    float (*red)[NW][DP] = (float (*)[NW][DP])red_;
    const int lane = threadIdx.x & 63, wave = threadIdx.x >> 6;
    float4 dg[NV], db[NV], gm[NV], cs[NV];
#pragma unroll
    for (int i = 0; i < NV; ++i) {
        dg[i] = db[i] = cs[i] = float4{0.f, 0.f, 0.f, 0.f};
        const int c = (i * 64 + lane) * 4;
        gm[i] = c < D ? *(const float4*)(gamma + c) : float4{0.f, 0.f, 0.f, 0.f};
    }
    struct Raw {
        float4 x[NV], a[NV], d[NV];
        float mu, rs;
        int64_t src;
        int row;
    };
    auto issue = [&](int row, Raw& r) {
        r.row = row;
        r.src = ridx ? ridx[row] : row;
        r.mu = mean[row];
        r.rs = rstd[row];
#pragma unroll
        for (int i = 0; i < NV; ++i) {
            const int c = (i * 64 + lane) * 4;
            r.x[i] = r.a[i] = r.d[i] = float4{0.f, 0.f, 0.f, 0.f};
            if (c < D) {
                r.x[i] = *(const float4*)(x + r.src * ldx + c);
                r.a[i] = *(const float4*)(dx_acc + r.src * lddx + c);
                if (DY_F32) r.d[i] = *(const float4*)((const float*)dy + (int64_t)row * lddy + c);
                else {
                    const bf16x4 t = *(const bf16x4*)((const bf16_t*)dy + (int64_t)row * lddy + c);
                    union { bf16x4 h; float2 f; } u; u.h = t;
                    r.d[i].x = u.f.x; r.d[i].y = u.f.y;
                }
            }
        }
    };
    auto process = [&](const Raw& r) {
        float4 xh[NV], g[NV];
        float s1 = 0.f, s2 = 0.f;
#pragma unroll
        for (int i = 0; i < NV; ++i) {
            const int c = (i * 64 + lane) * 4;
            xh[i] = g[i] = float4{0.f, 0.f, 0.f, 0.f};
            if (c < D) {
                float4 d;
                if (DY_F32) d = r.d[i];
                else {
                    union { bf16x4 h; float2 f; } u; u.f = float2{r.d[i].x, r.d[i].y};
                    d = float4{bf2f(u.h[0]), bf2f(u.h[1]), bf2f(u.h[2]), bf2f(u.h[3])};
                }
                const float4 xv = r.x[i];
                xh[i] = float4{(xv.x - r.mu) * r.rs, (xv.y - r.mu) * r.rs, (xv.z - r.mu) * r.rs, (xv.w - r.mu) * r.rs};
                g[i] = float4{d.x * gm[i].x, d.y * gm[i].y, d.z * gm[i].z, d.w * gm[i].w};
                s1 += (g[i].x + g[i].y) + (g[i].z + g[i].w);
                s2 += (g[i].x * xh[i].x + g[i].y * xh[i].y) + (g[i].z * xh[i].z + g[i].w * xh[i].w);
                dg[i].x += d.x * xh[i].x; dg[i].y += d.y * xh[i].y; dg[i].z += d.z * xh[i].z; dg[i].w += d.w * xh[i].w;
                db[i].x += d.x; db[i].y += d.y; db[i].z += d.z; db[i].w += d.w;
            }
        }
        const float c1 = wave_sum(s1) / D, c2 = wave_sum(s2) / D;
#pragma unroll
        for (int i = 0; i < NV; ++i) {
            const int c = (i * 64 + lane) * 4;
            if (c < D) {
                float* o = dx_acc + r.src * lddx + c;
                float4 a = r.a[i];
                a.x += r.rs * (g[i].x - c1 - xh[i].x * c2);
                a.y += r.rs * (g[i].y - c1 - xh[i].y * c2);
                a.z += r.rs * (g[i].z - c1 - xh[i].z * c2);
                a.w += r.rs * (g[i].w - c1 - xh[i].w * c2);
                *(float4*)o = a;
                cs[i].x += a.x; cs[i].y += a.y; cs[i].z += a.z; cs[i].w += a.w;
                if (dx_bf16) {
                    bf16x4 bq = {f2bf(a.x), f2bf(a.y), f2bf(a.z), f2bf(a.w)};
                    *(bf16x4*)(dx_bf16 + r.src * lddb + c) = bq;
                }
            }
        }
    };
    const int stride = gridDim.x * NW;
    Raw ra, rb;
    int row = blockIdx.x * NW + wave;
    if (row < M) issue(row, ra);
    while (row < M) {
        int nrow = row + stride;
        if (nrow < M) issue(nrow, rb);
        process(ra);
        row = nrow;
        if (row >= M) break;
        nrow = row + stride;
        if (nrow < M) issue(nrow, ra);
        process(rb);
        row = nrow;
    }
#pragma unroll
    for (int i = 0; i < NV; ++i) {
        const int c = (i * 64 + lane) * 4;
        *(float4*)&red[0][wave][c] = dg[i];
        *(float4*)&red[1][wave][c] = db[i];
        *(float4*)&red[2][wave][c] = cs[i];
    }
    __syncthreads();
    for (int c = threadIdx.x; c < D; c += 64 * NW) {
        float a = 0.f, b = 0.f, k = 0.f;
#pragma unroll
        for (int w = 0; w < NW; ++w) { a += red[0][w][c]; b += red[1][w][c]; k += red[2][w][c]; }
        if (dgamma) unsafeAtomicAdd(dgamma + c, a);
        if (dbeta) unsafeAtomicAdd(dbeta + c, b);
        if (colsum) unsafeAtomicAdd(colsum + c, k);
    }
}

}

#define LN_DISPATCH(NVV, ...)                     \
    switch (NVV) {                                \
        case 1: { constexpr int NV = 1; __VA_ARGS__; break; } \
        case 2: { constexpr int NV = 2; __VA_ARGS__; break; } \
        case 3: { constexpr int NV = 3; __VA_ARGS__; break; } \
        default: { constexpr int NV = 4; __VA_ARGS__; break; } \
    }

static int ln_fwd_launch(const void* x, int x_f16, int64_t ldx, const int32_t* row_index, const float* gamma, const float* beta, void* y,
                         int64_t ldy, int out, float* mean, float* rstd, int64_t M, int64_t D, float eps, void* stream, const char* who) {
    DCLIP_REQUIRE(x && gamma && beta && y, "%s: null operand", who);
    DCLIP_REQUIRE(M > 0, "%s: need M > 0 (M=%ld)", who, (long)M);
    DCLIP_REQUIRE(D > 0 && D % 4 == 0 && D <= 1024, "%s: need 0 < D <= 1024, D %% 4 == 0 (D=%ld)", who, (long)D);
    DCLIP_REQUIRE(out >= 0 && out <= 2 && (out != 2 || x_f16), "%s: output dtype 0 bf16 / 1 f32 (/ 2 f16 with f16 input)", who);
    DCLIP_REQUIRE(ldx % 4 == 0 && ldy % 4 == 0, "%s: row strides must be multiples of 4 (ldx=%ld, ldy=%ld)", who, (long)ldx, (long)ldy);
    DCLIP_REQUIRE(((uintptr_t)x % (x_f16 ? 8 : 16)) == 0, "%s: x must be %d-byte aligned", who, x_f16 ? 8 : 16);
    DCLIP_REQUIRE(((uintptr_t)y % (out == 1 ? 16 : 8)) == 0, "%s: y must be %d-byte aligned", who, out == 1 ? 16 : 8);
    DCLIP_REQUIRE((uintptr_t)gamma % 16 == 0 && (uintptr_t)beta % 16 == 0, "%s: gamma and beta must be 16-byte aligned", who);
    const int nv = (int)((D + 255) / 256);
    const dim3 grid((unsigned)((M + 3) / 4));
    hipStream_t st = (hipStream_t)stream;
    TraceScope tr(DCLIP_TRACE_LAYERNORM, 8.0 * (double)M * D, (double)M * D * ((x_f16 ? 2.0 : 4.0) + (out == 1 ? 4.0 : 2.0)), stream);
#define LN_GO(OUTV, XH) hipLaunchKernelGGL((ln_fwd_kernel<NV, OUTV, XH>), grid, dim3(256), 0, st, x, ldx, row_index, gamma, beta, y, ldy, mean, rstd, (int)M, (int)D, eps)
    LN_DISPATCH(nv,
        if (x_f16) { if (out == 2) LN_GO(2, true); else if (out == 1) LN_GO(1, true); else LN_GO(0, true); }
        else { if (out == 1) LN_GO(1, false); else LN_GO(0, false); });
#undef LN_GO
    return dclip_check_launch(who);
}

extern "C" int dclip_layernorm_fwd(const float* x, int64_t ldx, const int32_t* row_index, const float* gamma,
                                   const float* beta, void* y, int64_t ldy, int out_f32, float* mean, float* rstd,
                                   int64_t M, int64_t D, float eps, void* stream) {
    return ln_fwd_launch(x, 0, ldx, row_index, gamma, beta, y, ldy, out_f32, mean, rstd, M, D, eps, stream, "dclip_layernorm_fwd");
}

extern "C" int dclip_layernorm_fwd_f16(const void* x, int64_t ldx, const int32_t* row_index, const float* gamma,
                                       const float* beta, void* y, int64_t ldy, int out_dtype, float* mean, float* rstd,
                                       int64_t M, int64_t D, float eps, void* stream) {
    return ln_fwd_launch(x, 1, ldx, row_index, gamma, beta, y, ldy, out_dtype, mean, rstd, M, D, eps, stream, "dclip_layernorm_fwd_f16");
}

extern "C" int dclip_layernorm_bwd(const void* dy, int64_t lddy, int dy_f32, const float* x, int64_t ldx,
                                   const int32_t* row_index, const float* gamma, const float* mean, const float* rstd,
                                   float* dx_acc, int64_t lddx, void* dx_bf16, int64_t lddb, float* dgamma, float* dbeta,
                                   float* colsum_acc, int64_t M, int64_t D, void* stream) {
    DCLIP_REQUIRE(dy && x && gamma && mean && rstd && dx_acc, "dclip_layernorm_bwd: null operand");
    DCLIP_REQUIRE(M > 0, "dclip_layernorm_bwd: need M > 0 (M=%ld)", (long)M);
    DCLIP_REQUIRE(D > 0 && D % 4 == 0 && D <= 1024, "dclip_layernorm_bwd: need 0 < D <= 1024, D %% 4 == 0 (D=%ld)", (long)D);
    DCLIP_REQUIRE(lddy % 4 == 0 && ldx % 4 == 0 && lddx % 4 == 0 && (!dx_bf16 || lddb % 4 == 0),
                  "dclip_layernorm_bwd: row strides must be multiples of 4 (lddy=%ld, ldx=%ld, lddx=%ld, lddb=%ld)", (long)lddy, (long)ldx, (long)lddx, (long)lddb);
    DCLIP_REQUIRE(((uintptr_t)dy % (dy_f32 ? 16 : 8)) == 0, "dclip_layernorm_bwd: dy must be %d-byte aligned", dy_f32 ? 16 : 8);
    DCLIP_REQUIRE((uintptr_t)x % 16 == 0 && (uintptr_t)dx_acc % 16 == 0 && (uintptr_t)gamma % 16 == 0, "dclip_layernorm_bwd: x, dx_acc and gamma must be 16-byte aligned");
    DCLIP_REQUIRE((uintptr_t)dx_bf16 % 8 == 0, "dclip_layernorm_bwd: dx_bf16 must be 8-byte aligned");
    const int nv = (int)((D + 255) / 256);
    int blocks = (int)((M + 7) / 8);
    if (blocks > 256) blocks = 256;
    TraceScope tr(DCLIP_TRACE_LN_BWD, 12.0 * (double)M * D, (double)M * D * ((dy_f32 ? 4.0 : 2.0) + 12.0 + (dx_bf16 ? 2.0 : 0.0)), stream, (int)M, (int)D, 0, 0);
    hipStream_t st = (hipStream_t)stream;
    LN_DISPATCH(nv,
        if (dy_f32) hipLaunchKernelGGL((ln_bwd_kernel<NV, true>), dim3(blocks), dim3(512), (size_t)3 * 8 * NV * 256 * 4, st, dy, lddy, x, ldx, row_index, gamma, mean, rstd, dx_acc, lddx, (bf16_t*)dx_bf16, lddb, dgamma, dbeta, colsum_acc, (int)M, (int)D);
        else hipLaunchKernelGGL((ln_bwd_kernel<NV, false>), dim3(blocks), dim3(512), (size_t)3 * 8 * NV * 256 * 4, st, dy, lddy, x, ldx, row_index, gamma, mean, rstd, dx_acc, lddx, (bf16_t*)dx_bf16, lddb, dgamma, dbeta, colsum_acc, (int)M, (int)D));
    return dclip_check_launch("dclip_layernorm_bwd");
}
```

distillclip_amd/ops.py:

```python
import torch

from ._lib import lib

ACT = {'none': 0, None: 0, 'quickgelu': 1, 'gelu': 2, 'dgelu': 3, 'mulaux': 4, 'gelu_save': 5, 'quickgelu_save': 6}
OUT_DTYPE = {torch.bfloat16: 0, torch.float32: 1, torch.float16: 2}
DG_LO, DG_STEP = -0.13, 1.26 / 255.0


def _p(t):
    return 0 if t is None else t.data_ptr()


def _stream():
    return torch.cuda.current_stream().cuda_stream


def _chk(*ts):
    for t in ts:
        if t is not None and not t.is_cuda:
            raise RuntimeError('distillclip_amd ops need CUDA(HIP) tensors; there is no CPU fallback')


def gemm_nt(a, b, *, bias=None, act=None, aux_in=None, aux_out=None, residual=None, out=None, out_dtype=torch.bfloat16,
            alpha=1.0, row_group=0, rowadd=None, out_rows=None, colsum=None):
    _chk(a, b, bias, aux_in, aux_out, residual, out, rowadd)
    assert a.dtype == torch.bfloat16 and b.dtype == torch.bfloat16 and a.dim() == 2 and b.dim() == 2
    assert a.stride(1) == 1 and b.stride(1) == 1
    M, K = a.shape
    N = b.shape[0]
    if out is None:
        rows = out_rows if out_rows is not None else M
        out = torch.empty((rows, N), dtype=out_dtype, device=a.device)
    assert out.stride(1) == 1
    ldr = residual.stride(0) if residual is not None else 0
    if act in ('gelu_save', 'quickgelu_save') and aux_out is not None:
        assert aux_out.dtype == torch.uint8 and aux_out.stride(0) == out.stride(0)
    if act == 'mulaux':
        assert aux_in.dtype == torch.uint8 and aux_in.stride(0) == out.stride(0)
    if residual is not None:
        assert residual.dtype == (torch.float16 if out.dtype == torch.float16 else torch.float32)
    lib().dclip_gemm_nt(_p(a), a.stride(0), _p(b), b.stride(0), _p(out), out.stride(0), M, N, K, float(alpha),
                        _p(bias), ACT[act], _p(aux_in), _p(aux_out), _p(residual), ldr,
                        OUT_DTYPE[out.dtype], row_group, _p(rowadd), _p(colsum), _stream())
    return out


_TN_WS = {}


def _tn_workspace(device):
    key = (device, _stream())
    ws = _TN_WS.get(key)
    if ws is None:
        ws = _TN_WS[key] = torch.empty(lib().dclip_gemm_tn_workspace_bytes(), dtype=torch.uint8, device=device)
    return ws


def gemm_tn_acc(a, b, dw, splits=4, workspace=True):
    _chk(a, b, dw)
    assert a.dtype == torch.bfloat16 and b.dtype == torch.bfloat16 and dw.dtype == torch.float32
    M, P = a.shape
    Q = b.shape[1]
    assert b.shape[0] == M and tuple(dw.shape) == (P, Q) and dw.stride(1) == 1
    ws = _tn_workspace(a.device) if workspace else None
    lib().dclip_gemm_tn_acc(_p(a), a.stride(0), _p(b), b.stride(0), _p(dw), dw.stride(0), M, P, Q, splits, _p(ws),
                            0 if ws is None else ws.numel(), _stream())
    return dw


def colsum_acc(x, db):
    _chk(x, db)
    assert x.dtype == torch.bfloat16 and db.dtype == torch.float32
    lib().dclip_colsum_acc(_p(x), x.stride(0), _p(db), x.shape[0], x.shape[1], _stream())
    return db


def layernorm_fwd(x, gamma, beta, *, row_index=None, out_dtype=torch.bfloat16, eps=1e-5, save_stats=True):
    _chk(x, gamma, beta, row_index)
    assert x.dtype in (torch.float32, torch.float16) and x.dim() == 2 and x.stride(1) == 1
    M = row_index.numel() if row_index is not None else x.shape[0]
    D = x.shape[1]
    y = torch.empty((M, D), dtype=out_dtype, device=x.device)
    mean = torch.empty(M, dtype=torch.float32, device=x.device) if save_stats else None
    rstd = torch.empty(M, dtype=torch.float32, device=x.device) if save_stats else None
    fn = lib().dclip_layernorm_fwd_f16 if x.dtype == torch.float16 else lib().dclip_layernorm_fwd
    fn(_p(x), x.stride(0), _p(row_index), _p(gamma), _p(beta), _p(y), D, OUT_DTYPE[out_dtype], _p(mean), _p(rstd), M, D, eps, _stream())
    return y, mean, rstd


def layernorm_bwd(dy, x, gamma, mean, rstd, dx_acc, *, row_index=None, dx_bf16=None, dgamma=None, dbeta=None, colsum=None):
    _chk(dy, x, gamma, mean, rstd, dx_acc, dx_bf16, dgamma, dbeta)
    M, D = dy.shape
    lib().dclip_layernorm_bwd(_p(dy), dy.stride(0), 1 if dy.dtype == torch.float32 else 0, _p(x), x.stride(0),
                              _p(row_index), _p(gamma), _p(mean), _p(rstd), _p(dx_acc), dx_acc.stride(0), _p(dx_bf16),
                              dx_bf16.stride(0) if dx_bf16 is not None else 0, _p(dgamma), _p(dbeta), _p(colsum), M, D, _stream())


def attn_nt(a, lda, bm, ldb, B, H, N, hd, alpha=1.0, out_dtype=torch.float32):
    Np = (N + 7) // 8 * 8
    c = torch.empty((B, H, N, Np), dtype=out_dtype, device=a.device)
    lib().dclip_attn_nt(_p(a), lda, _p(bm), ldb, _p(c), 1 if out_dtype == torch.float32 else 0, B, H, N, Np, hd, alpha,
                        _stream())
    return c


def _score_dims(a):
    if a.dim() == 5:
        B, H, nq, N, four = a.shape
        assert four == 4
        return B, H, N, nq * 4, 1
    B, H, N, Np = a.shape
    return B, H, N, Np, 0


def attn_nn(a, bm, ldb, c, ldc, hd, alpha=1.0):
    B, H, N, Np, blocked = _score_dims(a)
    lib().dclip_attn_nn(_p(a), _p(bm), ldb, _p(c), ldc, B, H, N, Np, hd, alpha, blocked, _stream())


def attn_tn(a, bm, ldb, c, ldc, hd, alpha=1.0):
    B, H, N, Np, blocked = _score_dims(a)
    lib().dclip_attn_tn(_p(a), _p(bm), ldb, _p(c), ldc, B, H, N, Np, hd, alpha, blocked, _stream())


def attn_nn_rows(a, bm, ldb, c, ldc, hd, pick, alpha=1.0, fill_zero=False):
    _chk(pick)
    B, H, N, Np, blocked = _score_dims(a)
    lib().dclip_attn_nn_rows(_p(a), _p(bm), ldb, _p(c), ldc, B, H, N, Np, hd, alpha, blocked, _p(pick), 1 if fill_zero else 0, _stream())


def attn_tn_rows(a, bm, ldb, c, ldc, hd, pick, alpha=1.0):
    _chk(pick)
    B, H, N, Np, blocked = _score_dims(a)
    lib().dclip_attn_tn_rows(_p(a), _p(bm), ldb, _p(c), ldc, B, H, N, Np, hd, alpha, blocked, _p(pick), _stream())


def unblock_scores(a):
    B, H, nq, N, _ = a.shape
    return a.permute(0, 1, 3, 2, 4).reshape(B, H, N, nq * 4)


def attn_softmax_fwd(s, wl=None, ww=None, causal=False, save_p=False):
    B, H, N, Np = s.shape
    r = torch.empty((B, H, N, Np), dtype=torch.bfloat16, device=s.device)
    p = torch.empty_like(r) if save_p else None
    lib().dclip_attn_softmax_fwd(_p(s), _p(wl), _p(ww), _p(p), _p(r), B, H, N, Np, 1 if causal else 0, _stream())
    return p, r


def attn_softmax_bwd(dr, p, s, wl=None, ww=None, dwl=None, dww=None):
    B, H, N, Np = dr.shape
    ds = torch.empty_like(dr)
    lib().dclip_attn_softmax_bwd(_p(dr), _p(p), _p(s), 1 if (s is not None and s.dtype == torch.bfloat16) else 0, _p(wl), _p(ww), _p(ds),
                                 _p(dwl), _p(dww), B, H, N, Np, _stream())
    return ds


LOSS_SLOTS = {'out_l1': 0, 'out_cos': 1, 'out_kl': 2, 'out_ce': 3, 'cos_diff': 4, 'hard_label': 5, 'soft_label': 6,
              'logits_mse': 7}


def distill_loss(s_img, t_img, s_txt=None, t_txt=None, *, weights, temperature=None, row0=None, rows=None, gathered_stats=None,
                 stats_only=False):
    import ctypes
    _chk(s_img, t_img, s_txt, t_txt)
    B, E = s_img.shape
    two = s_txt is not None
    cfg = [0.0] * 10
    for k, w in weights.items():
        cfg[LOSS_SLOTS[k]] = float(w)
    cfg[8] = float(temperature or 0.0)
    cfg[9] = 1.0 if two else 0.0
    cfg_arr = (ctypes.c_float * 10)(*cfg)
    ws_bytes = lib().dclip_distill_loss_workspace(B, E)
    ws = torch.empty(ws_bytes, dtype=torch.uint8, device=s_img.device)
    out = torch.empty(16, dtype=torch.float32, device=s_img.device)
    nrow = B if rows is None else int(rows)
    d_i = torch.empty((nrow, E), dtype=torch.float32, device=s_img.device)
    d_t = torch.empty((nrow, E), dtype=torch.float32, device=s_img.device) if two else None
    if rows is None:
        lib().dclip_distill_loss(_p(s_img), _p(t_img), _p(s_txt), _p(t_txt), B, E, ctypes.cast(cfg_arr, ctypes.c_void_p),
                                 _p(out), _p(d_i), _p(d_t), _p(ws), ws_bytes, _stream())
    else:
        stats = torch.empty((6, nrow), dtype=torch.float32, device=s_img.device) if stats_only else None
        if gathered_stats is not None:
            assert gathered_stats.shape == (6, B) and gathered_stats.dtype == torch.float32 and gathered_stats.is_contiguous()
        lib().dclip_distill_loss_rows(_p(s_img), _p(t_img), _p(s_txt), _p(t_txt), B, E, int(row0), nrow,
                                      ctypes.cast(cfg_arr, ctypes.c_void_p), _p(out), _p(d_i), _p(d_t), _p(gathered_stats),
                                      _p(stats), _p(ws), ws_bytes, _stream())
        if stats_only:
            return stats
    return out, d_i, d_t


def interactive_loss(s_img, t_img, s_txt, t_txt, temperature, weight=1.0):
    _chk(s_img, t_img, s_txt, t_txt)
    for t in (s_img, t_img, s_txt, t_txt):
        if t.dtype != torch.float32 or t.dim() != 2 or t.shape != s_img.shape or not t.is_contiguous():
            raise ValueError(f'interactive_loss: need four contiguous f32 [B, E] tensors of one shape, got {tuple(t.shape)} {t.dtype}')
    B, E = s_img.shape
    ws_bytes = lib().dclip_interactive_loss_workspace(B, E)
    if ws_bytes == 0:
        raise ValueError(f'interactive_loss: need 1 <= B <= 4096, E % 16 == 0, 16 <= E <= 1024, got B={B} E={E}')
    ws = torch.empty(ws_bytes, dtype=torch.uint8, device=s_img.device)
    out = torch.empty(4, dtype=torch.float32, device=s_img.device)
    d_i, d_t = torch.empty_like(s_img), torch.empty_like(s_txt)
    lib().dclip_interactive_loss(_p(s_img), _p(t_img), _p(s_txt), _p(t_txt), B, E, float(temperature), float(weight), _p(out), _p(d_i),
                                 _p(d_t), _p(ws), ws_bytes, _stream())
    return out, d_i, d_t


def attn_fused_fwd(qkv, B, N, H, hd, causal=False):
    _chk(qkv)
    D = H * hd
    ctx = torch.empty((B * N, D), dtype=torch.bfloat16, device=qkv.device)
    lib().dclip_attn_fused_fwd(_p(qkv), qkv.stride(0), _p(ctx), D, B, H, N, hd, hd ** -0.5, 1 if causal else 0, _stream())
    return ctx


def attn_fused_fwd_rows(qkv, ctx, B, N, H, hd, pick, causal=False):
    _chk(qkv, ctx, pick)
    lib().dclip_attn_fused_fwd_rows(_p(qkv), qkv.stride(0), _p(ctx), ctx.stride(0), B, H, N, hd, hd ** -0.5, 1 if causal else 0, _p(pick),
                                    _stream())
    return ctx


def attn_stream_fwd(qkv, B, N, H, hd):
    _chk(qkv)
    D = H * hd
    ctx = torch.empty((B * N, D), dtype=torch.bfloat16, device=qkv.device)
    lib().dclip_attn_stream_fwd(_p(qkv), qkv.stride(0), _p(ctx), D, B, H, N, hd, hd ** -0.5, _stream())
    return ctx


def im2row_ld(image, patch, ldk=None, cls_rows=1):
    _chk(image)
    assert image.dtype == torch.float32 and image.dim() == 4 and image.is_contiguous() and image.shape[2] == image.shape[3]
    B, C, R, _ = image.shape
    K = C * patch * patch
    ldk = (K + 63) // 64 * 64 if ldk is None else int(ldk)
    g = R // patch
    rows = torch.empty((B * (g * g + cls_rows), ldk), dtype=torch.bfloat16, device=image.device)
    lib().dclip_im2row_ld(_p(image), _p(rows), ldk, B, C, R, patch, cls_rows, _stream())
    return rows


def embed_scatter_add(ids, dx, dtable):
    _chk(ids, dx, dtable)
    rows, D = dx.shape
    lib().dclip_embed_scatter_add(_p(ids), _p(dx), 1 if dx.dtype == torch.float32 else 0, _p(dtable), rows, D, dtable.shape[0],
                                  _stream())
    return dtable


def feature_mse(s, t, coef=1.0):
    _chk(s, t)
    assert s.dtype == torch.float32 and t.dtype == torch.float32 and s.numel() == t.numel() and s.numel() % 4 == 0
    val = torch.zeros(1, dtype=torch.float32, device=s.device)
    ds = torch.zeros_like(s)
    lib().dclip_feature_mse(_p(s), _p(t), s.numel(), float(coef), _p(val), _p(ds), _stream())
    return val[0], ds


def attn_mix_fwd(qkv, B, N, H, hd, wl, ww, scale):
    _chk(qkv, wl, ww)
    Np = (N + 7) // 8 * 8
    r = torch.full((B, H, Np // 4, N, 4), float('nan'), dtype=torch.bfloat16, device=qkv.device)
    stats = torch.empty((B, H, N), dtype=torch.float32, device=qkv.device)
    lib().dclip_attn_mix_fwd(_p(qkv), qkv.stride(0), _p(wl), _p(ww), _p(r), _p(stats), B, H, N, Np, hd, scale, _stream())
    return r, stats


def attn_mix_bwd(qkv, d_ctx, B, N, H, hd, wl, ww, stats, scale, dwl, dww):
    _chk(qkv, d_ctx, wl, ww, stats, dwl, dww)
    Np = (N + 7) // 8 * 8
    ds = torch.full((B, H, Np // 4, N, 4), float('nan'), dtype=torch.bfloat16, device=qkv.device)
    ws = torch.empty(lib().dclip_attn_mix_bwd_workspace_bytes(B, H, N), dtype=torch.uint8, device=qkv.device)
    lib().dclip_attn_mix_bwd(_p(qkv), qkv.stride(0), _p(d_ctx), d_ctx.stride(0), _p(wl), _p(ww), _p(stats), _p(ds), _p(dwl), _p(dww),
                             _p(ws), ws.numel(), B, H, N, Np, hd, scale, _stream())
    return ds


def attn_mix_fwd_rows(qkv, r, stats, wl, ww, scale, pick):
    _chk(qkv, r, stats, wl, ww, pick)
    B, H, N, Np, _ = _score_dims(r)
    lib().dclip_attn_mix_fwd_rows(_p(qkv), qkv.stride(0), _p(wl), _p(ww), _p(r), _p(stats), B, H, N, Np, qkv.shape[1] // (3 * H), scale,
                                  _p(pick), _stream())


def attn_mix_bwd_rows(qkv, d_ctx, ds, wl, ww, stats, scale, dwl, dww, pick, ws=None):
    _chk(qkv, d_ctx, ds, wl, ww, stats, dwl, dww, pick)
    B, H, N, Np, _ = _score_dims(ds)
    if ws is None:
        ws = torch.empty(lib().dclip_attn_mix_bwd_workspace_bytes(B, H, N), dtype=torch.uint8, device=qkv.device)
    lib().dclip_attn_mix_bwd_rows(_p(qkv), qkv.stride(0), _p(d_ctx), d_ctx.stride(0), _p(wl), _p(ww), _p(stats), _p(ds), _p(dwl), _p(dww),
                                  _p(ws), ws.numel(), B, H, N, Np, qkv.shape[1] // (3 * H), scale, _p(pick), _stream())


def cast_transpose_multi(ws, want_b=True, want_t=True):
    import ctypes
    _chk(*ws)
    n = len(ws)
    wb = [torch.empty_like(w, dtype=torch.bfloat16) for w in ws] if want_b else [None] * n
    wt = [torch.empty((w.shape[1], w.shape[0]), dtype=torch.bfloat16, device=w.device) for w in ws] if want_t else [None] * n
    arr = lambda ts: (ctypes.c_void_p * n)(*[None if t is None else t.data_ptr() for t in ts])
    R = (ctypes.c_int64 * n)(*[w.shape[0] for w in ws])
    C = (ctypes.c_int64 * n)(*[w.shape[1] for w in ws])
    lib().dclip_cast_transpose_bf16_multi(arr(ws), arr(wb), arr(wt), R, C, n, _stream())
    return (wb if want_b else None), (wt if want_t else None)


SUMSQ_PARTIALS = 1024
ADAMW_MAX_RANGES = 24


def _range_arrays(items, width):
    import ctypes
    for it in items:
        _chk(*it)
    n = len(items)
    ptrs = [(ctypes.c_void_p * max(n, 1))(*[t[k].data_ptr() for t in items]) for k in range(width)]
    return ptrs, (ctypes.c_int64 * max(n, 1))(*[t[0].numel() for t in items]), n


def sumsq_multi(gs, partials, stream=None):
    _chk(partials)
    (ptrs,), lens, n = _range_arrays([(g,) for g in gs], 1)
    lib().dclip_sumsq_multi(ptrs, lens, n, _p(partials), partials.numel(), _stream() if stream is None else stream)
    return partials


def clip_coef(partials, max_norm, out, extra_sumsq=None, stream=None):
    _chk(partials, extra_sumsq, out)
    lib().dclip_clip_coef(_p(partials), partials.numel(), _p(extra_sumsq), float(max_norm), _p(out), _stream() if stream is None else stream)
    return out


def adamw_multi_scaled(items, lr, betas, eps, weight_decay, step, zero_grad=False, gscale=None, stream=None):
    ptrs, lens, n = _range_arrays(items, 4)
    _chk(gscale)
    lib().dclip_adamw_multi_scaled(*ptrs, lens, n, lr, betas[0], betas[1], eps, weight_decay, step,
                                   1 if zero_grad else 0, _p(gscale), _stream() if stream is None else stream)


AMP_RECORD_FLOATS = 8
AMP_MULT, AMP_SKIP, AMP_BC1, AMP_BC2_SQRT, AMP_NORM, AMP_COEF = range(6)


def amp_prepare(record, skipped, betas, step, found_inf=None, grad_scale=None, partials=None, max_norm=0.0, extra_sumsq=None, stream=None):
    _chk(record, skipped, found_inf, grad_scale, partials, extra_sumsq)
    for t in (found_inf, grad_scale):
        if t is not None and (t.dtype != torch.float32 or t.numel() != 1):
            raise ValueError('amp_prepare: found_inf and grad_scale are 1-element f32 tensors')
    if record.dtype != torch.float32 or record.numel() < AMP_RECORD_FLOATS or skipped.dtype != torch.int64:
        raise ValueError('amp_prepare: record is %d f32, skipped one int64' % AMP_RECORD_FLOATS)
    lib().dclip_amp_prepare(_p(found_inf), _p(grad_scale), _p(partials), 0 if partials is None else partials.numel(), _p(extra_sumsq), float(max_norm),
                            betas[0], betas[1], step, _p(skipped), _p(record), _stream() if stream is None else stream)
    return record


def adamw_multi_amp(items, lr, betas, eps, weight_decay, zero_grad, record, stream=None):
    ptrs, lens, n = _range_arrays(items, 4)
    _chk(record)
    lib().dclip_adamw_multi_amp(*ptrs, lens, n, lr, betas[0], betas[1], eps, weight_decay, 1 if zero_grad else 0,
                                _p(record), _stream() if stream is None else stream)


def adamw_multi_ema(items, lr, betas, eps, weight_decay, step, zero_grad, ema_weight, gscale=None, record=None, stream=None):
    ptrs, lens, n = _range_arrays(items, 5)
    _chk(gscale, record)
    lib().dclip_adamw_multi_ema(*ptrs, lens, n, lr, betas[0], betas[1], eps, weight_decay, step,
                                1 if zero_grad else 0, ema_weight, _p(gscale), _p(record), _stream() if stream is None else stream)


ADAMW_TABLE_TILE = 8192


def adamw_table_image(ranges, total, out=None):
    import ctypes
    n = len(ranges)
    need = lib().dclip_adamw_table_bytes(n)
    if out is None:
        out = torch.zeros(max(need, 8), dtype=torch.uint8)
    if out.is_cuda or out.dtype != torch.uint8 or not out.is_contiguous():
        raise ValueError('adamw_table_image: out is a contiguous CPU uint8 tensor')
    col = lambda k, ct: (ct * max(n, 1))(*[r[k] for r in ranges])
    tiles = ctypes.c_int64(0)
    lib().dclip_adamw_table_fill(col(0, ctypes.c_int64), col(1, ctypes.c_int64), col(2, ctypes.c_float), col(3, ctypes.c_float), n, total,
                                 out.data_ptr(), out.numel(), ctypes.byref(tiles))
    return out, tiles.value


def _table_operands(what, p, g, m, v, e, table, count):
    if table.dtype != torch.uint8 or table.numel() < lib().dclip_adamw_table_bytes(count):
        raise ValueError('%s: table is the uint8 device copy of an image of %d ranges' % (what, count))
    if any(t.numel() != p.numel() or t.dtype != torch.float32 for t in (p, g, m, v) + (() if e is None else (e,))):
        raise ValueError('%s: p, g, m, v (and e) are f32 buffers of one length, the `total` the table was filled for' % what)


def adamw_table(p, g, m, v, e, table, count, tiles, lr, betas, eps, step, zero_grad=False, ema_weight=0.0, gscale=None, record=None, stream=None):
    _chk(p, g, m, v, e, table, gscale, record)
    _table_operands('adamw_table', p, g, m, v, e, table, count)
    lib().dclip_adamw_table(_p(p), _p(g), _p(m), _p(v), _p(e), _p(table), count, tiles, lr, betas[0], betas[1], eps, step, 1 if zero_grad else 0,
                            ema_weight, _p(gscale), _p(record), _stream() if stream is None else stream)


def lamb_buffers(count, tiles, device):
    return (torch.empty(max(lib().dclip_lamb_workspace_bytes(count, tiles), 16), dtype=torch.uint8, device=device),
            torch.zeros(count, 4, dtype=torch.float32, device=device))


def lamb_table(p, g, m, v, e, table, count, tiles, lr, betas, eps, step, workspace, stats, zero_grad=False, ema_weight=0.0, gscale=None, record=None,
               trust_clip=None, always_adapt=False, stream=None):
    _chk(p, g, m, v, e, table, gscale, record, workspace, stats)
    _table_operands('lamb_table', p, g, m, v, e, table, count)
    if workspace.dtype != torch.uint8 or stats.dtype != torch.float32 or stats.numel() < 4 * count:
        raise ValueError('lamb_table: workspace is uint8, stats f32 [%d, 4] (lamb_buffers)' % count)
    lib().dclip_lamb_table(_p(p), _p(g), _p(m), _p(v), _p(e), _p(table), count, tiles, lr, betas[0], betas[1], eps, step, 1 if zero_grad else 0,
                           ema_weight, _p(gscale), _p(record), -1.0 if trust_clip is None else float(trust_clip), 1 if always_adapt else 0,
                           _p(workspace), workspace.numel(), _p(stats), _stream() if stream is None else stream)


def swap_multi(pairs, stream=None):
    for a, b in pairs:
        _chk(a, b)
        if a.numel() != b.numel():
            raise ValueError('swap_multi: the two sides of a pair have %d and %d elements' % (a.numel(), b.numel()))
    ptrs, lens, n = _range_arrays(pairs, 2)
    lib().dclip_swap_multi(*ptrs, lens, n, _stream() if stream is None else stream)


def clipscore(img, cand, refs=None, ref_offsets=None, *, K=1, w=2.5):
    _chk(img, cand, refs, ref_offsets)
    if (refs is None) != (ref_offsets is None):
        raise ValueError('clipscore: refs and ref_offsets come together')
    for name, t in (('img', img), ('cand', cand), ('refs', refs)):
        if t is not None and (t.dtype != torch.float32 or t.dim() != 2 or t.stride(1) != 1):
            raise ValueError(f'clipscore: {name} must be an f32 [rows, E] matrix with unit column stride')
    B, E = img.shape
    K = int(K)
    if K < 1 or cand.shape != (B * K, E) or (refs is not None and refs.shape[1] != E):
        raise ValueError(f'clipscore: img {tuple(img.shape)} and K={K} need cand [{B * K}, {E}] and refs [R, {E}], got {tuple(cand.shape)}'
                         + ('' if refs is None else f' and {tuple(refs.shape)}'))
    R = 0
    if refs is not None:
        if ref_offsets.dtype != torch.int32 or ref_offsets.dim() != 1 or ref_offsets.numel() != B + 1 or not ref_offsets.is_contiguous():
            raise ValueError(f'clipscore: ref_offsets must be a contiguous int32 [{B + 1}] tensor')
        R = refs.shape[0]
        if R == 0:
            refs = img.new_zeros((1, E))
    clip_s = torch.empty(B * K, dtype=torch.float32, device=img.device)
    ref_s = torch.empty_like(clip_s) if refs is not None else None
    refclip_s = torch.empty_like(clip_s) if refs is not None else None
    lib().dclip_clipscore(_p(img), img.stride(0), _p(cand), cand.stride(0), _p(refs), 0 if refs is None else refs.stride(0),
                          _p(ref_offsets), B, K, R, E, float(w), _p(clip_s), _p(ref_s), _p(refclip_s), _stream())
    return clip_s, ref_s, refclip_s
```

include/dclip.h:

```cpp
#ifndef DCLIP_H
#define DCLIP_H
#include <stddef.h>
#include <stdint.h>
#ifdef __cplusplus
extern "C" {
#endif

#define DCLIP_OK 0
#define DCLIP_EINVAL (-1)
#define DCLIP_ELAUNCH (-2)

int dclip_version(void);
int dclip_runtime_check(void);
const char* dclip_arch(void);
const char* dclip_last_error_string(void);

#define DCLIP_ACT_NONE 0
#define DCLIP_ACT_QUICKGELU 1
#define DCLIP_ACT_GELU 2
#define DCLIP_ACT_DGELU 3
#define DCLIP_ACT_MULAUX 4
#define DCLIP_ACT_GELU_SAVE 5
#define DCLIP_ACT_QUICKGELU_SAVE 6
#define DCLIP_OUT_BF16 0
#define DCLIP_OUT_F32 1
#define DCLIP_OUT_F16 2

int dclip_gemm_nt(const void* A, int64_t lda, const void* B, int64_t ldb, void* C, int64_t ldc,
                  int64_t M, int64_t N, int64_t K, float alpha, const float* bias, int act,
                  const void* aux_in, void* aux_out, const void* residual, int64_t ldr, int out_dtype,
                  int64_t row_group, const float* rowadd, float* colsum_acc, void* stream);

size_t dclip_gemm_tn_workspace_bytes(void);
int64_t dclip_gemm_tn_atomic_fallbacks(void);
int dclip_gemm_tn_acc(const void* A, int64_t lda, const void* B, int64_t ldb, float* dW, int64_t ldo,
                      int64_t M, int64_t P, int64_t Q, int splits, void* workspace, size_t ws_bytes, void* stream);

int dclip_colsum_acc(const void* X, int64_t ld, float* db, int64_t M, int64_t N, void* stream);

int dclip_layernorm_fwd(const float* x, int64_t ldx, const int32_t* row_index, const float* gamma, const float* beta,
                        void* y, int64_t ldy, int out_f32, float* mean, float* rstd, int64_t M, int64_t D, float eps,
                        void* stream);
int dclip_layernorm_fwd_f16(const void* x, int64_t ldx, const int32_t* row_index, const float* gamma, const float* beta,
                            void* y, int64_t ldy, int out_dtype, float* mean, float* rstd, int64_t M, int64_t D, float eps,
                            void* stream);
int dclip_layernorm_bwd(const void* dy, int64_t lddy, int dy_f32, const float* x, int64_t ldx, const int32_t* row_index,
                        const float* gamma, const float* mean, const float* rstd, float* dx_acc, int64_t lddx,
                        void* dx_bf16, int64_t lddb, float* dgamma, float* dbeta, float* colsum_acc, int64_t M, int64_t D,
                        void* stream);

int dclip_attn_nt(const void* A, int64_t lda, const void* Bm, int64_t ldb, void* C, int out_f32, int64_t B, int64_t H,
                  int64_t N, int64_t Np, int64_t hd, float alpha, void* stream);
int dclip_attn_nn(const void* A, const void* Bm, int64_t ldb, void* C, int64_t ldc, int64_t B, int64_t H, int64_t N,
                  int64_t Np, int64_t hd, float alpha, int a_blocked, void* stream);
int dclip_attn_tn(const void* A, const void* Bm, int64_t ldb, void* C, int64_t ldc, int64_t B, int64_t H, int64_t N,
                  int64_t Np, int64_t hd, float alpha, int a_blocked, void* stream);
int dclip_attn_fused_fwd(const void* qkv, int64_t ldq, void* ctx, int64_t ldc, int64_t B, int64_t H, int64_t N, int64_t hd,
                         float scale, int causal, void* stream);
int dclip_attn_stream_fwd(const void* qkv, int64_t ldq, void* ctx, int64_t ldc, int64_t B, int64_t H, int64_t N, int64_t hd,
                          float scale, void* stream);
int dclip_attn_softmax_fwd(const float* S, const float* Wl, const float* Ww, void* P, void* R, int64_t B, int64_t H,
                           int64_t N, int64_t Np, int causal, void* stream);
int dclip_attn_softmax_bwd(const void* dR, const void* P, const void* S, int scores_bf16, const float* Wl, const float* Ww,
                           void* dS, float* dWl, float* dWw, int64_t B, int64_t H, int64_t N, int64_t Np, void* stream);
int dclip_attn_mix_supported(int64_t H, int64_t N, int64_t hd);
size_t dclip_attn_mix_bwd_workspace_bytes(int64_t B, int64_t H, int64_t N);
void dclip_attn_mix_debug_stamps(void* fwd, void* bwd_a, void* bwd_b);
int dclip_attn_mix_fwd(const void* qkv, int64_t ld, const float* Wl, const float* Ww, void* R, float* stats, int64_t B, int64_t H,
                       int64_t N, int64_t Np, int64_t hd, float scale, void* stream);
int dclip_attn_mix_bwd(const void* qkv, int64_t ld, const void* dO, int64_t ldo, const float* Wl, const float* Ww,
                       const float* stats, void* dS, float* dWl, float* dWw, void* workspace, size_t ws_bytes, int64_t B, int64_t H,
                       int64_t N, int64_t Np, int64_t hd, float scale, void* stream);
int dclip_attn_nn_rows(const void* A, const void* Bm, int64_t ldb, void* C, int64_t ldc, int64_t B, int64_t H, int64_t N, int64_t Np,
                       int64_t hd, float alpha, int a_blocked, const int32_t* pick, int fill_zero, void* stream);
int dclip_attn_tn_rows(const void* A, const void* Bm, int64_t ldb, void* C, int64_t ldc, int64_t B, int64_t H, int64_t N, int64_t Np,
                       int64_t hd, float alpha, int a_blocked, const int32_t* pick, void* stream);
int dclip_attn_fused_fwd_rows(const void* qkv, int64_t ldq, void* ctx, int64_t ldc, int64_t B, int64_t H, int64_t N, int64_t hd,
                              float scale, int causal, const int32_t* pick, void* stream);
int dclip_attn_mix_fwd_rows(const void* qkv, int64_t ld, const float* Wl, const float* Ww, void* R, float* stats, int64_t B, int64_t H,
                            int64_t N, int64_t Np, int64_t hd, float scale, const int32_t* pick, void* stream);
int dclip_attn_mix_bwd_rows(const void* qkv, int64_t ld, const void* dO, int64_t ldo, const float* Wl, const float* Ww,
                            const float* stats, void* dS, float* dWl, float* dWw, void* workspace, size_t ws_bytes, int64_t B, int64_t H,
                            int64_t N, int64_t Np, int64_t hd, float scale, const int32_t* pick, void* stream);
int dclip_attn_maps_fwd(const void* qkv, int64_t ld, const float* Wl, float* score_map, float* prob_map, int64_t B, int64_t H, int64_t N,
                        int64_t hd, float scale, int causal, void* stream);
size_t dclip_attn_maps_bwd_workspace_bytes(int64_t B, int64_t H, int64_t N);
int dclip_attn_maps_bwd(const void* qkv, int64_t ld, const float* Wl, const float* d_score_map, const float* d_prob_map, void* dS,
                        int ds_blocked, float* dWl, void* workspace, size_t ws_bytes, int64_t B, int64_t H, int64_t N, int64_t Np,
                        int64_t hd, float scale, int causal, void* stream);

int dclip_cast_bf16(const float* src, void* dst, int64_t n, void* stream);
int dclip_cast_f16_f32(const void* src, float* dst, int64_t n, void* stream);
int dclip_axpy_f32(float* dst, const float* src, void* dst_bf16, int64_t n, float* colsum_acc, int64_t D, void* stream);
int dclip_cast_transpose_bf16_multi(const float* const* W, void* const* Wb, void* const* Wt, const int64_t* R, const int64_t* C,
                                    int64_t n, void* stream);
int dclip_im2row(const float* img, void* rows, int64_t B, int64_t C, int64_t res, int64_t patch, int cls_rows, void* stream);
int dclip_im2row_ld(const float* img, void* rows, int64_t ldk, int64_t B, int64_t C, int64_t res, int64_t patch, int cls_rows,
                    void* stream);
int dclip_token_table(const float* pos, const float* cls, const float* bias, float* out, int64_t ntok, int64_t D, void* stream);
int dclip_token_table_bwd(const float* tok_sum, float* dpos, float* dcls, float* dbias, int64_t ntok, int64_t D, int has_cls,
                          void* stream);
int dclip_batch_sum_acc(const float* G, float* out, int64_t B, int64_t N, int64_t D, void* stream);
int dclip_embed_gather(const int64_t* ids, int64_t id_stride, const float* table, const float* pos, void* out, int out_dtype,
                       int64_t rows, int64_t N, int64_t D, void* stream);
int dclip_embed_scatter_add(const int64_t* ids, const void* dx, int dx_f32, float* dtable, int64_t rows, int64_t D,
                            int64_t vocab, void* stream);
int dclip_pick_index(const int64_t* ids, int64_t id_stride, int32_t* idx, int64_t B, int64_t N, void* stream);
int dclip_adamw(float* p, float* g, float* m, float* v, int64_t n, float lr, float beta1, float beta2, float eps,
                float weight_decay, int64_t step, int zero_grad, void* stream);
#define DCLIP_ADAMW_MAX_RANGES 24
int dclip_adamw_multi(float* const* p, float* const* g, float* const* m, float* const* v, const int64_t* n, int32_t count, float lr,
                      float beta1, float beta2, float eps, float weight_decay, int64_t step, int zero_grad, void* stream);
int dclip_adamw_multi_scaled(float* const* p, float* const* g, float* const* m, float* const* v, const int64_t* n, int32_t count,
                             float lr, float beta1, float beta2, float eps, float weight_decay, int64_t step, int zero_grad,
                             const float* gscale, void* stream);
#define DCLIP_SUMSQ_PARTIALS 1024
int dclip_sumsq_multi(const float* const* g, const int64_t* n, int32_t count, float* partials, int64_t n_partials, void* stream);
int dclip_clip_coef(const float* partials, int64_t n_partials, const float* extra_sumsq, float max_norm, float* out, void* stream);
#define DCLIP_AMP_RECORD_FLOATS 8
#define DCLIP_AMP_MULT 0
#define DCLIP_AMP_SKIP 1
#define DCLIP_AMP_BC1 2
#define DCLIP_AMP_BC2_SQRT 3
#define DCLIP_AMP_NORM 4
#define DCLIP_AMP_COEF 5
int dclip_amp_prepare(const float* found_inf, const float* grad_scale, const float* partials, int64_t n_partials, const float* extra_sumsq,
                      float max_norm, float beta1, float beta2, int64_t step, int64_t* skipped, float* record, void* stream);
int dclip_adamw_multi_amp(float* const* p, float* const* g, float* const* m, float* const* v, const int64_t* n, int32_t count, float lr,
                          float beta1, float beta2, float eps, float weight_decay, int zero_grad, const float* record, void* stream);
int dclip_adamw_multi_ema(float* const* p, float* const* g, float* const* m, float* const* v, float* const* e, const int64_t* n, int32_t count,
                          float lr, float beta1, float beta2, float eps, float weight_decay, int64_t step, int zero_grad, float ema_weight,
                          const float* gscale, const float* record, void* stream);
int dclip_swap_multi(float* const* a, float* const* b, const int64_t* n, int32_t count, void* stream);
#define DCLIP_ADAMW_TABLE_TILE 8192
typedef struct dclip_adamw_range {
    int64_t tile0;
    int64_t begin, length;
    float lr_scale, weight_decay;
} dclip_adamw_range;
size_t dclip_adamw_table_bytes(int32_t count);
int dclip_adamw_table_fill(const int64_t* begin, const int64_t* length, const float* lr_scale, const float* weight_decay, int32_t count,
                           int64_t total, void* image, size_t image_bytes, int64_t* tiles);
int dclip_adamw_table(float* p, float* g, float* m, float* v, float* e, const void* table, int32_t count, int64_t tiles, float lr, float beta1,
                      float beta2, float eps, int64_t step, int zero_grad, float ema_weight, const float* gscale, const float* record,
                      void* stream);
size_t dclip_lamb_workspace_bytes(int32_t count, int64_t tiles);
int dclip_lamb_table(float* p, float* g, float* m, float* v, float* e, const void* table, int32_t count, int64_t tiles, float lr, float beta1,
                     float beta2, float eps, int64_t step, int zero_grad, float ema_weight, const float* gscale, const float* record,
                     float trust_clip, int always_adapt, void* workspace, size_t ws_bytes, float* stats, void* stream);

size_t dclip_distill_loss_workspace(int64_t B, int64_t E);
int dclip_distill_loss(const float* s_img, const float* t_img, const float* s_txt, const float* t_txt, int64_t B, int64_t E,
                       const float* cfg, float* out_scalars, float* d_s_img, float* d_s_txt, void* workspace,
                       size_t ws_bytes, void* stream);
typedef struct dclip_aug_op {
    int32_t op;
    int32_t c[6];
    float f;
} dclip_aug_op;
size_t dclip_augment_workspace(int64_t B, int64_t H, int64_t W);
int dclip_augment_normalize(const uint8_t* images, int64_t B, int64_t H, int64_t W, const dclip_aug_op* ops, int num_ops,
                            const float* mean3, const float* std3, float* out, uint8_t* aug_out, void* workspace,
                            size_t ws_bytes, void* stream);
typedef struct dclip_resize_desc {
    int64_t src_offset;
    int64_t table_offset;
    int64_t temp_offset;
    int32_t height, width;
    int32_t row0, nrows;
    int32_t ksize_h, ksize_v;
} dclip_resize_desc;
int dclip_resize_center_crop(const uint8_t* packed, const dclip_resize_desc* desc, const int32_t* tables, int64_t B, int64_t S,
                             uint8_t* out, void* workspace, size_t ws_bytes, void* stream);
size_t dclip_retrieval_metrics_workspace(int64_t n, int64_t E);
int dclip_retrieval_metrics(const float* img, const float* txt, int64_t n, int64_t E, const int32_t* ks, int nk,
                            float* out, int32_t* rank_out, void* workspace, size_t ws_bytes, void* stream);
size_t dclip_retrieval_recall_workspace(int64_t n_img, int64_t n_txt, int64_t E);
int dclip_retrieval_recall(const float* img, const float* txt, const int32_t* txt_offsets, int64_t n_img, int64_t n_txt, int64_t E,
                           const int32_t* ks, int nk, float* out, int32_t* rank_i2t, int32_t* rank_t2i, void* workspace, size_t ws_bytes,
                           void* stream);
size_t dclip_topk_search_workspace(int64_t nq, int64_t ng, int64_t E, int k);
int dclip_topk_search(const float* queries, const float* gallery, int64_t nq, int64_t ng, int64_t E, int k, int32_t* idx, float* score,
                      void* workspace, size_t ws_bytes, void* stream);
int dclip_group_mean_rows(const float* rows, const int32_t* offsets, int64_t n_groups, int64_t n_rows, int64_t E, float* out,
                          void* stream);
int dclip_clipscore(const float* img, int64_t ld_img, const float* cand, int64_t ld_cand, const float* refs, int64_t ld_ref,
                    const int32_t* ref_offsets, int64_t B, int64_t K, int64_t R, int64_t E, float w, float* clip_s, float* ref_s,
                    float* refclip_s, void* stream);
size_t dclip_kendall_tau_workspace(int64_t n, int64_t C);
int dclip_kendall_tau(const float* scores, int64_t ld, int64_t C, const float* human, int64_t n, double* out_tau, int64_t* out_counts,
                      void* workspace, size_t ws_bytes, void* stream);
size_t dclip_rank_correlation_workspace(int64_t n, int64_t C);
int dclip_rank_correlation(const float* scores, int64_t ld, int64_t C, const float* human, int64_t n, double* out_corr, int64_t* out_sums,
                           int32_t* out_ranks, void* workspace, size_t ws_bytes, void* stream);
int dclip_distill_loss_rows(const float* s_img, const float* t_img, const float* s_txt, const float* t_txt, int64_t B, int64_t E,
                            int64_t row0, int64_t rows, const float* cfg, float* out_scalars, float* d_s_img, float* d_s_txt,
                            const float* gathered_stats, float* stats_out, void* workspace, size_t ws_bytes, void* stream);
int dclip_feature_mse(const float* s, const float* t, int64_t n, float coef, float* loss_acc, float* ds_acc, void* stream);
size_t dclip_interactive_loss_workspace(int64_t B, int64_t E);
int dclip_interactive_loss(const float* s_img, const float* t_img, const float* s_txt, const float* t_txt, int64_t B, int64_t E,
                           float tau, float weight, float* out, float* d_s_img, float* d_s_txt, void* workspace, size_t ws_bytes,
                           void* stream);

typedef struct dclip_encoder_cfg {
    int32_t kind;
    int32_t modality;
    int32_t tokens;
    int32_t width;
    int32_t heads;
    int32_t layers;
    int32_t repeats;
    int32_t mlp_dim;
    int32_t out_dim;
    int32_t patch, resolution, in_chans;
    int32_t vocab, embed_rank;
    int32_t head_mix;
    int32_t causal;
} dclip_encoder_cfg;

typedef struct dclip_encoder dclip_encoder;

dclip_encoder* dclip_encoder_create(const dclip_encoder_cfg* cfg);
void dclip_encoder_destroy(dclip_encoder* enc);
int64_t dclip_encoder_num_params(const dclip_encoder* enc);
size_t dclip_encoder_wcache_bytes(const dclip_encoder* enc);
size_t dclip_encoder_workspace_bytes(const dclip_encoder* enc, int64_t B, int training);
int dclip_encoder_prepare(const dclip_encoder* enc, const void* const* params, void* wcache, void* stream);
typedef struct dclip_attn_maps {
    int32_t n;
    const int32_t* exec;
    float* const* score;
    float* const* prob;
    const float* const* d_score;
    const float* const* d_prob;
    void* scratch;
    size_t scratch_bytes;
} dclip_attn_maps;
typedef struct dclip_encoder_run {
    uint32_t flags;
    uint32_t reserved;
    uint64_t score_maps;
    uint64_t prob_maps;
} dclip_encoder_run;
int dclip_encoder_forward(const dclip_encoder* enc, const void* input, const void* patches, int64_t B, const void* const* params,
                          const void* wcache, void* workspace, size_t ws_bytes, dclip_encoder_run* run, int training,
                          float* last_representation, float* const* rep_out, float* emb_out, int64_t tokens_eff,
                          const dclip_attn_maps* maps, void* stream);
size_t dclip_encoder_last_layer_output_scratch_bytes(const dclip_encoder* enc, int64_t B, int training);
int dclip_encoder_last_layer_output(const dclip_encoder* enc, int64_t B, const void* const* params, const void* wcache,
                                    void* workspace, size_t ws_bytes, const dclip_encoder_run* run, int training, void* scratch,
                                    float* out, void* stream);
typedef void (*dclip_bucket_cb)(void* user, int32_t bucket);
int dclip_encoder_backward(const dclip_encoder* enc, const void* input, const void* patches, int64_t B, const void* const* params,
                           void* const* grads, const void* wcache, void* workspace, size_t ws_bytes, dclip_encoder_run* run,
                           const float* d_last_representation, const float* const* d_rep, const float* d_emb,
                           const dclip_attn_maps* maps, dclip_bucket_cb on_bucket, void* cb_user, void* stream);
int32_t dclip_encoder_num_grad_buckets(const dclip_encoder* enc);
int dclip_encoder_grad_bucket(const dclip_encoder* enc, int32_t bucket, int32_t* first_param, int32_t* end_param);

int dclip_trace_begin(int64_t max_records);
int64_t dclip_trace_end(int32_t* kind, float* ms, double* flops, double* bytes, int64_t cap);
int64_t dclip_trace_dims(int32_t* dims, int64_t cap);
int dclip_trace_gemm_stamps(void* buf);
int dclip_trace_attn_stamps(void* buf);
int64_t dclip_trace_gemm_clock(void* buf, int64_t cap);

#ifdef __cplusplus
}
#endif
#endif
```

Measured before the change: 18680 pairs/s.

## Fuse qkv bias colsum into weight-grad GEMM and seed LN backward from compact grads

Folds the qkv bias-gradient column sum into the 256-tile TN weight-gradient GEMM. It does this with an extra MFMA against a ones vector, writing per-split partials that the existing reduce kernel sums. It also replaces the separate rows_expand of the compact residual gradient with a seeded layernorm-backward kernel that reads the compact gradient via the pick index. It adds a ragged-M tail path for the TN kernel. This removes a colsum pass over dqkv and a full M×D fp32 expand copy, at the cost of extra MFMA work and template variants that may raise register pressure.

```diff
diff --git a/distillclip_amd/csrc/encoder.cpp b/distillclip_amd/csrc/encoder.cpp
--- a/distillclip_amd/csrc/encoder.cpp
+++ b/distillclip_amd/csrc/encoder.cpp
@@ -700,17 +700,24 @@
             bf16_t* dctx_c = dqkv;
             CK(gemm(gb_pr, D, W + bw.proj_t, D, dctx_c, D, B, D, D, nullptr, 0, nullptr, nullptr, nullptr, 0, DCLIP_OUT_BF16, 0, nullptr, st));
             CK(dclip_rows_expand(dctx_c, dctx, w.pick, B, N, D * 2, st));
-            CK(dclip_rows_expand(w.Gc, w.G, w.pick, B, N, D * 4, st));
         }
         const MapGrad mg{gm.score[ei], gm.prob[ei], maps ? maps->scratch : nullptr, maps ? maps->scratch_bytes : 0};
         CK(attn_backward(w.path, p, s, w, wl, ww, gl, gw, dctx, dqkv, B, mg.d_score || mg.d_prob ? &mg : nullptr,
                          compact && (run->flags & RUN_PRUNED_ATTN) ? w.pick : nullptr, st));
-        if (r == 0 && GR(bx.qkvw)) CK(dclip_gemm_tn_acc(w.dqkv, 3 * D, s0.h1, D, GR(bx.qkvw), D, MR, 3 * D, D, wsplits(MR, 3 * D, D), w.tn_ws, w.tn_ws_bytes, st));
-        if (r == 0 && params[bx.qkvb] && GR(bx.qkvb)) CK(dclip_colsum_acc(w.dqkv, 3 * D, GR(bx.qkvb), MR, 3 * D, st));
+        float* g_qkvb = r == 0 && params[bx.qkvb] ? GR(bx.qkvb) : nullptr;
+        if (r == 0 && GR(bx.qkvw) && g_qkvb)
+            CK(dclip_gemm_tn_acc_colsum(w.dqkv, 3 * D, s0.h1, D, GR(bx.qkvw), D, g_qkvb, MR, 3 * D, D, wsplits(MR, 3 * D, D), 0, w.tn_ws, w.tn_ws_bytes, st));
+        else {
+            if (r == 0 && GR(bx.qkvw)) CK(dclip_gemm_tn_acc(w.dqkv, 3 * D, s0.h1, D, GR(bx.qkvw), D, MR, 3 * D, D, wsplits(MR, 3 * D, D), w.tn_ws, w.tn_ws_bytes, st));
+            if (g_qkvb) CK(dclip_colsum_acc(w.dqkv, 3 * D, g_qkvb, MR, 3 * D, st));
+        }
         CK(gemm(dqkv, 3 * D, W + bw.qkv_t, 3 * D, w.dh, D, M, D, 3 * D, nullptr, 0, nullptr, nullptr, nullptr, 0, DCLIP_OUT_BF16, 0, nullptr, st));
         bf16_t* gb_next = ei > 0 ? w.gb_f2 + (int64_t)((ei - 1) % R) * M * D : w.Gb;
-        CK(dclip_layernorm_bwd(w.dh, D, 0, (const float*)w.X[ei], D, nullptr, PF(params, bx.n1w), s.mean1, s.rstd1, w.G, D, gb_next, D, GR(bx.n1w), GR(bx.n1b),
-                               ei > 0 ? GR(bexec(p, (ei - 1) / p.R, 0).f2b) : nullptr, M, D, st));
+        float* db_prev = ei > 0 ? GR(bexec(p, (ei - 1) / p.R, 0).f2b) : nullptr;
+        if (compact) CK(dclip_layernorm_bwd_seeded(w.dh, D, 0, (const float*)w.X[ei], D, PF(params, bx.n1w), s.mean1, s.rstd1, w.Gc, w.pick, B, N, w.G, D,
+                                                   gb_next, D, GR(bx.n1w), GR(bx.n1b), db_prev, D, st));
+        else CK(dclip_layernorm_bwd(w.dh, D, 0, (const float*)w.X[ei], D, nullptr, PF(params, bx.n1w), s.mean1, s.rstd1, w.G, D, gb_next, D, GR(bx.n1w), GR(bx.n1b),
+                                    db_prev, M, D, st));
         if (r == 0 && on_bucket) on_bucket(cb_user, 1 + (p.L - 1 - l));
     }
 
diff --git a/distillclip_amd/csrc/gemm_tn.hip b/distillclip_amd/csrc/gemm_tn.hip
--- a/distillclip_amd/csrc/gemm_tn.hip
+++ b/distillclip_amd/csrc/gemm_tn.hip
@@ -18,6 +18,7 @@
     int tiles_p, tiles_q, splits, chunk;
     unsigned long long* stamps;
     float* partial;
+    float* csum_partial;
 };
 
 __device__ __forceinline__ void tn_load(const bf16_t* __restrict__ G, int64_t ld, int m0, int m_end, int c0, int cols,
@@ -148,6 +149,17 @@
 #pragma unroll
     for (int s = 0; s < NP; ++s)
         __builtin_amdgcn_global_load_lds((gbl_void*)(src[s] + chunk_off), (lds_void*)(tile + (wave * NP + s) * 1024), 16, 0, 0);
+}
+
+__device__ u32x4 tn_zero16[1];
+template <int NP>
+__device__ __forceinline__ void tn_stage_tail(const char* const (&src)[NP], int64_t chunk_off, char* tile, int wave, int lane, int rows) {
+#pragma unroll
+    for (int s = 0; s < NP; ++s) {
+        const int piece = wave * NP + s;
+        const char* g = piece * 4 + (lane >> 4) < rows ? src[s] + chunk_off : (const char*)tn_zero16;
+        __builtin_amdgcn_global_load_lds((gbl_void*)g, (lds_void*)(tile + piece * 1024), 16, 0, 0);
+    }
 }
 
 template <int OFF>
@@ -224,16 +236,34 @@
     }
 }
 
-__global__ __launch_bounds__(512) void gemm_tn256_kernel(GemmTN p) {
-    extern __shared__ __attribute__((aligned(16))) char smem[];
+#define TN_PHASE_MFMA_CS(acc, R0, af, b0, b1, cs, wc, ones)                                                               \
+    do {                                                                                                                  \
+        __builtin_amdgcn_s_barrier();                                                                                     \
+        __builtin_amdgcn_s_setprio(1);                                                                                    \
+        _Pragma("unroll") for (int kb_ = 0; kb_ < 2; ++kb_)                                                               \
+            _Pragma("unroll") for (int i_ = 0; i_ < 4; ++i_) {                                                            \
+                _Pragma("unroll") for (int j_ = 0; j_ < 2; ++j_)                                                          \
+                    acc[(R0) + i_][j_] = mfma_rc<false>(af[i_][kb_], b0[j_][kb_], acc[(R0) + i_][j_]);                    \
+                _Pragma("unroll") for (int j_ = 0; j_ < 2; ++j_)                                                          \
+                    acc[(R0) + i_][2 + j_] = mfma_rc<false>(af[i_][kb_], b1[j_][kb_], acc[(R0) + i_][2 + j_]);            \
+            }                                                                                                             \
+        _Pragma("unroll") for (int kb_ = 0; kb_ < 2; ++kb_) {                                                             \
+            cs = mfma_rc<false>(af[(wc)][kb_], ones, cs);                                                                 \
+        }                                                                                                                 \
+        __builtin_amdgcn_s_setprio(0);                                                                                    \
+        __builtin_amdgcn_s_barrier();                                                                                     \
+    } while (0)
+
+template <bool CSUM, bool RAGGED, int WC>
+__device__ __forceinline__ void tn256_body(const GemmTN& p, char* smem) {
     const int tid = threadIdx.x, lane = tid & 63;
     const int wave = __builtin_amdgcn_readfirstlane(tid >> 6);
-    const int wr = wave >> 2, wc = wave & 3;
+    const int wr = wave >> 2, wc = WC >= 0 ? WC : wave & 3;
 
     const TnWork w = tn_locate<256>(p);
     const int p0 = w.p0, q0 = w.q0, m_begin = w.m_begin, m_end = w.m_end;
     if (m_begin >= m_end) return;
-    const int nk = (m_end - m_begin) / TC;
+    const int nk = RAGGED ? (m_end - m_begin + TC - 1) / TC : (m_end - m_begin) / TC;
     const int nload = 4 * nk;
 
     f32x4 acc[8][4];
@@ -251,6 +281,14 @@
     auto issue = [&](int l) {
         const int kt = l >> 2, hw = l & 3;
         char* buf = smem + ((kt & 1) * 4 + hw) * HT;
+        if (RAGGED && m_begin + (kt + 1) * TC > m_end) {
+            const int rows = m_end - m_begin - kt * TC;
+            if (hw == 0) tn_stage_tail(srcs[0], kt * step_b, buf, wave, lane, rows);
+            else if (hw == 1) tn_stage_tail(srcs[1], kt * step_b, buf, wave, lane, rows);
+            else if (hw == 2) tn_stage_tail(srcs[2], kt * step_a, buf, wave, lane, rows);
+            else tn_stage_tail(srcs[3], kt * step_a, buf, wave, lane, rows);
+            return;
+        }
         if (hw == 0) tn_stage(srcs[0], kt * step_b, buf, wave);
         else if (hw == 1) tn_stage(srcs[1], kt * step_b, buf, wave);
         else if (hw == 2) tn_stage(srcs[2], kt * step_a, buf, wave);
@@ -270,6 +308,11 @@
     const int b_off = (wc >> 1) * HT;
     const int bcol = (wc & 1) * 64;
     bf16x8 af[4][2], b0[2][2], b1[2][2];
+    f32x4 csa = f32x4{0.f, 0.f, 0.f, 0.f}, csb = csa;
+    bf16x8 ones;
+#pragma unroll
+    for (int e = 0; e < 8; ++e) ones[e] = (bf16_t)1.f;
+    if constexpr (CSUM) asm volatile("" : "+v"(ones));
 
     for (int kt = 0; kt < nk; ++kt) {
         const char* base = smem + (kt & 1) * 4 * HT;
@@ -292,7 +335,8 @@
         if (k4 + 7 < nload) issue(k4 + 7);
         WAIT_LGKM0();
         __builtin_amdgcn_sched_barrier(0);
-        PHASE_MFMA(false, acc, 0, 4, af, b0, b1);
+        if constexpr (CSUM) TN_PHASE_MFMA_CS(acc, 0, af, b0, b1, csa, WC, ones);
+        else PHASE_MFMA(false, acc, 0, 4, af, b0, b1);
         __builtin_amdgcn_sched_barrier(0);
 #pragma unroll
         for (int i = 0; i < 4; ++i) {
@@ -303,10 +347,17 @@
         else WAIT_VMCNT(0);
         WAIT_LGKM0();
         __builtin_amdgcn_sched_barrier(0);
-        PHASE_MFMA(false, acc, 4, 4, af, b0, b1);
+        if constexpr (CSUM) TN_PHASE_MFMA_CS(acc, 4, af, b0, b1, csb, WC, ones);
+        else PHASE_MFMA(false, acc, 4, 4, af, b0, b1);
     }
     if (wr == 0) __builtin_amdgcn_s_barrier();
     wg_stamp(p.stamps, tid, 2);
+
+    if (CSUM && q0 == 0 && (lane & 15) == 0) {
+        float* row = p.csum_partial + (int64_t)w.split * p.P + p0 + wr * 128 + wc * 16 + (lane >> 4) * 4;
+        *(float4*)row = float4{csa[0], csa[1], csa[2], csa[3]};
+        *(float4*)(row + 64) = float4{csb[0], csb[1], csb[2], csb[3]};
+    }
 
     float* cs = (float*)smem;
     constexpr int CL = 256 + 4;
@@ -334,10 +385,35 @@
         }
     }
     wg_stamp(p.stamps, tid, 3);
+    if constexpr (CSUM) mfma_keep_alive(ones);
+}
+
+template <bool CSUM, bool RAGGED>
+__global__ __launch_bounds__(512) void gemm_tn256_kernel(GemmTN p) {
+    extern __shared__ __attribute__((aligned(16))) char smem[];
+    if constexpr (CSUM) {
+        switch (__builtin_amdgcn_readfirstlane(threadIdx.x >> 6) & 3) {
+            case 0: tn256_body<true, RAGGED, 0>(p, smem); break;
+            case 1: tn256_body<true, RAGGED, 1>(p, smem); break;
+            case 2: tn256_body<true, RAGGED, 2>(p, smem); break;
+            default: tn256_body<true, RAGGED, 3>(p, smem); break;
+        }
+    } else {
+        tn256_body<false, RAGGED, -1>(p, smem);
+    }
 }
 
 __global__ __launch_bounds__(256) void tn256_reduce_kernel(const float* __restrict__ partial, int splits, int tiles, int tiles_q,
-                                                           float* __restrict__ out, int64_t ldo) {
+                                                           float* __restrict__ out, int64_t ldo, const float* __restrict__ csum_partial,
+                                                           int P, float* __restrict__ db) {
+    if ((int)blockIdx.x >= tiles * 64) {
+        const int c = ((int)blockIdx.x - tiles * 64) * 256 + threadIdx.x;
+        if (c >= P) return;
+        float a = csum_partial[c];
+        for (int s = 1; s < splits; ++s) a += csum_partial[(int64_t)s * P + c];
+        db[c] += a;
+        return;
+    }
     const int idx = blockIdx.x * 256 + threadIdx.x;
     const int tile = idx >> 14, rt = (idx >> 6) & 255, c4 = idx & 63;
     if (tile >= tiles) return;
@@ -424,42 +500,70 @@
 
 extern "C" size_t dclip_gemm_tn_workspace_bytes(void) { return (size_t)384 * 65536 * sizeof(float); }
 
-extern "C" int dclip_gemm_tn_acc(const void* A, int64_t lda, const void* B, int64_t ldb, float* dW, int64_t ldo,
-                                 int64_t M, int64_t P, int64_t Q, int splits, void* workspace, size_t ws_bytes, void* stream) {
-    DCLIP_REQUIRE(A && B && dW, "dclip_gemm_tn_acc: null operand");
-    DCLIP_REQUIRE(M > 0 && P > 0 && Q > 0, "dclip_gemm_tn_acc: empty problem");
+extern "C" int dclip_colsum_acc(const void* X, int64_t ld, float* db, int64_t M, int64_t N, void* stream);
+
+static int gemm_tn_launch(const void* A, int64_t lda, const void* B, int64_t ldb, float* dW, int64_t ldo, float* dA_colsum, int64_t M, int64_t P,
+                          int64_t Q, int splits, int tile256, void* workspace, size_t ws_bytes, void* stream, const char* who) {
+    DCLIP_REQUIRE(A && B && dW, "%s: null operand", who);
+    DCLIP_REQUIRE(M > 0 && P > 0 && Q > 0, "%s: empty problem", who);
     DCLIP_REQUIRE(P % 8 == 0 && Q % 8 == 0 && lda % 8 == 0 && ldb % 8 == 0 &&
                   ((uintptr_t)A % 16) == 0 && ((uintptr_t)B % 16) == 0,
-                  "dclip_gemm_tn_acc: P, Q, lda, ldb must be multiples of 8 and bases 16-byte aligned");
-    DCLIP_REQUIRE(splits >= 1, "dclip_gemm_tn_acc: splits must be >= 1");
+                  "%s: P, Q, lda, ldb must be multiples of 8 and bases 16-byte aligned", who);
+    DCLIP_REQUIRE(splits >= 1, "%s: splits must be >= 1", who);
+    DCLIP_REQUIRE(!tile256 || (P % 256 == 0 && Q % 256 == 0 && M < (1LL << 31) - 64), "%s: the 256 x 256 pipeline needs P %% 256 == 0 and Q %% 256 == 0", who);
     GemmTN p;
     p.A = (const bf16_t*)A; p.lda = lda; p.B = (const bf16_t*)B; p.ldb = ldb; p.out = dW; p.ldo = ldo;
-    p.M = (int)M; p.P = (int)P; p.Q = (int)Q; p.stamps = g_gemm_stamps; p.partial = nullptr;
+    p.M = (int)M; p.P = (int)P; p.Q = (int)Q; p.stamps = g_gemm_stamps; p.partial = nullptr; p.csum_partial = nullptr;
     const bool fast = M % TC == 0 && P >= 8 && Q >= 8;
-    const bool big = fast && P % 256 == 0 && Q % 256 == 0 && (P / 256) * (Q / 256) >= 16 && M >= 4096;
+    const bool big = tile256 || (fast && P % 256 == 0 && Q % 256 == 0 && (P / 256) * (Q / 256) >= 16 && M >= 4096);
     TraceScope tr(DCLIP_TRACE_GEMM_TN, 2.0 * (double)M * (double)P * (double)Q, 2.0 * ((double)M * P + (double)M * Q) + 4.0 * (double)P * Q, stream, (int)M, (int)P, (int)Q, big ? 256 : 128);
     if (big) {
         p.tiles_p = (int)(P / 256); p.tiles_q = (int)(Q / 256);
         const int tiles = p.tiles_p * p.tiles_q;
-        const int s = (256 + tiles / 2) / tiles;
+        const int s = tile256 ? splits : (256 + tiles / 2) / tiles;
         set_splits(p, s < 1 ? 1 : s);
         static const int tn_partial = [] { const char* e = getenv("DCLIP_TN_PARTIAL"); return e ? atoi(e) : 1; }();
-        const size_t need = (size_t)tiles * p.splits * 65536 * sizeof(float);
-        const bool part = tn_partial != 0 && workspace && ws_bytes >= need && ldo % 4 == 0 && ((uintptr_t)dW % 16) == 0 && p.splits > 1;
+        const size_t tile_bytes = (size_t)tiles * p.splits * 65536 * sizeof(float);
+        const size_t need = tile_bytes + (dA_colsum ? (size_t)p.splits * P * sizeof(float) : 0);
+        const bool part = tn_partial != 0 && workspace && ws_bytes >= need && ldo % 4 == 0 && ((uintptr_t)dW % 16) == 0 &&
+                          ((uintptr_t)workspace % 16) == 0 && (p.splits > 1 || dA_colsum);
         if (!part && p.splits > 1) g_tn_atomic_fallbacks.fetch_add(1, std::memory_order_relaxed);
         p.partial = part ? (float*)workspace : nullptr;
-        hipLaunchKernelGGL(gemm_tn256_kernel, dim3(tiles * p.splits), dim3(512), 8 * HT, (hipStream_t)stream, p);
+        const bool csum = part && dA_colsum;
+        if (csum) p.csum_partial = (float*)((char*)workspace + tile_bytes);
+        const dim3 grid(tiles * p.splits);
+        if (M % TC != 0) {
+            if (csum) hipLaunchKernelGGL((gemm_tn256_kernel<true, true>), grid, dim3(512), 8 * HT, (hipStream_t)stream, p);
+            else hipLaunchKernelGGL((gemm_tn256_kernel<false, true>), grid, dim3(512), 8 * HT, (hipStream_t)stream, p);
+        } else if (csum) hipLaunchKernelGGL((gemm_tn256_kernel<true, false>), grid, dim3(512), 8 * HT, (hipStream_t)stream, p);
+        else hipLaunchKernelGGL((gemm_tn256_kernel<false, false>), grid, dim3(512), 8 * HT, (hipStream_t)stream, p);
         if (part)
-            hipLaunchKernelGGL(tn256_reduce_kernel, dim3((unsigned)(tiles * 64)), dim3(256), 0, (hipStream_t)stream, (const float*)workspace,
-                               p.splits, tiles, p.tiles_q, dW, ldo);
-        return dclip_check_launch("dclip_gemm_tn_acc");
+            hipLaunchKernelGGL(tn256_reduce_kernel, dim3((unsigned)(tiles * 64 + (csum ? (P + 255) / 256 : 0))), dim3(256), 0, (hipStream_t)stream,
+                               (const float*)workspace, p.splits, tiles, p.tiles_q, dW, ldo, (const float*)p.csum_partial, (int)P, dA_colsum);
+        const int rc = dclip_check_launch(who);
+        if (rc != DCLIP_OK || !dA_colsum || csum) return rc;
+        return dclip_colsum_acc(A, lda, dA_colsum, M, P, stream);
     }
     p.tiles_p = (int)((P + TP - 1) / TP); p.tiles_q = (int)((Q + TQ - 1) / TQ);
     set_splits(p, splits);
     const int grid = p.tiles_p * p.tiles_q * p.splits;
     if (fast) hipLaunchKernelGGL(gemm_tn_glds_kernel, dim3(grid), dim3(256), TN_LDS, (hipStream_t)stream, p);
     else hipLaunchKernelGGL(gemm_tn_kernel, dim3(grid), dim3(256), 4 * TTILE, (hipStream_t)stream, p);
-    return dclip_check_launch("dclip_gemm_tn_acc");
+    const int rc = dclip_check_launch(who);
+    if (rc != DCLIP_OK || !dA_colsum) return rc;
+    return dclip_colsum_acc(A, lda, dA_colsum, M, P, stream);
+}
+
+extern "C" int dclip_gemm_tn_acc(const void* A, int64_t lda, const void* B, int64_t ldb, float* dW, int64_t ldo,
+                                 int64_t M, int64_t P, int64_t Q, int splits, void* workspace, size_t ws_bytes, void* stream) {
+    return gemm_tn_launch(A, lda, B, ldb, dW, ldo, nullptr, M, P, Q, splits, 0, workspace, ws_bytes, stream, "dclip_gemm_tn_acc");
+}
+
+extern "C" int dclip_gemm_tn_acc_colsum(const void* A, int64_t lda, const void* B, int64_t ldb, float* dW, int64_t ldo, float* dA_colsum,
+                                        int64_t M, int64_t P, int64_t Q, int splits, int tile256, void* workspace, size_t ws_bytes,
+                                        void* stream) {
+    DCLIP_REQUIRE(dA_colsum, "dclip_gemm_tn_acc_colsum: null operand");
+    return gemm_tn_launch(A, lda, B, ldb, dW, ldo, dA_colsum, M, P, Q, splits, tile256 != 0, workspace, ws_bytes, stream, "dclip_gemm_tn_acc_colsum");
 }
 
 extern "C" int dclip_colsum_acc(const void* X, int64_t ld, float* db, int64_t M, int64_t N, void* stream) {
diff --git a/distillclip_amd/csrc/layernorm.hip b/distillclip_amd/csrc/layernorm.hip
--- a/distillclip_amd/csrc/layernorm.hip
+++ b/distillclip_amd/csrc/layernorm.hip
@@ -64,13 +64,15 @@
     }
 }
 
-template <int NV, bool DY_F32>
+template <int NV, bool DY_F32, bool SEEDED = false>
 __global__ __launch_bounds__(512) void ln_bwd_kernel(const void* __restrict__ dy, int64_t lddy, const float* __restrict__ x,
                                                      int64_t ldx, const int* __restrict__ ridx,
                                                      const float* __restrict__ gamma, const float* __restrict__ mean,
                                                      const float* __restrict__ rstd, float* __restrict__ dx_acc,
                                                      int64_t lddx, bf16_t* __restrict__ dx_bf16, int64_t lddb,
-                                                     float* __restrict__ dgamma, float* __restrict__ dbeta, float* __restrict__ colsum, int M, int D) {
+                                                     float* __restrict__ dgamma, float* __restrict__ dbeta, float* __restrict__ colsum, int M, int D,
+                                                     const float* __restrict__ seed = nullptr, const int* __restrict__ seed_pick = nullptr,
+                                                     int seed_n = 1) {
     constexpr int NW = 8, DP = NV * 256;
     extern __shared__ float red_[];
     float (*red)[NW][DP] = (float (*)[NW][DP])red_;
@@ -93,13 +95,19 @@
         r.src = ridx ? ridx[row] : row;
         r.mu = mean[row];
         r.rs = rstd[row];
+        int sb = -1;
+        if (SEEDED) {
+            const int b = (int)r.src / seed_n;
+            if (seed_pick[b] == (int)r.src) sb = b;
+        }
 #pragma unroll
         for (int i = 0; i < NV; ++i) {
             const int c = (i * 64 + lane) * 4;
             r.x[i] = r.a[i] = r.d[i] = float4{0.f, 0.f, 0.f, 0.f};
             if (c < D) {
                 r.x[i] = *(const float4*)(x + r.src * ldx + c);
-                r.a[i] = *(const float4*)(dx_acc + r.src * lddx + c);
+                if (!SEEDED) r.a[i] = *(const float4*)(dx_acc + r.src * lddx + c);
+                else if (sb >= 0) r.a[i] = *(const float4*)(seed + (int64_t)sb * D + c);
                 if (DY_F32) r.d[i] = *(const float4*)((const float*)dy + (int64_t)row * lddy + c);
                 else {
                     const bf16x4 t = *(const bf16x4*)((const bf16_t*)dy + (int64_t)row * lddy + c);
@@ -229,25 +237,46 @@
     return ln_fwd_launch(x, 1, ldx, row_index, gamma, beta, y, ldy, out_dtype, mean, rstd, M, D, eps, stream, "dclip_layernorm_fwd_f16");
 }
 
+static int ln_bwd_launch(const void* dy, int64_t lddy, int dy_f32, const float* x, int64_t ldx, const int32_t* row_index, const float* gamma,
+                         const float* mean, const float* rstd, float* dx_acc, int64_t lddx, void* dx_bf16, int64_t lddb, float* dgamma,
+                         float* dbeta, float* colsum_acc, int64_t M, int64_t D, const float* seed, const int32_t* seed_pick, int64_t seed_n,
+                         void* stream, const char* who) {
+    DCLIP_REQUIRE(dy && x && gamma && mean && rstd && dx_acc, "%s: null operand", who);
+    DCLIP_REQUIRE(M > 0, "%s: need M > 0 (M=%ld)", who, (long)M);
+    DCLIP_REQUIRE(D > 0 && D % 4 == 0 && D <= 1024, "%s: need 0 < D <= 1024, D %% 4 == 0 (D=%ld)", who, (long)D);
+    DCLIP_REQUIRE(lddy % 4 == 0 && ldx % 4 == 0 && lddx % 4 == 0 && (!dx_bf16 || lddb % 4 == 0),
+                  "%s: row strides must be multiples of 4 (lddy=%ld, ldx=%ld, lddx=%ld, lddb=%ld)", who, (long)lddy, (long)ldx, (long)lddx, (long)lddb);
+    DCLIP_REQUIRE(((uintptr_t)dy % (dy_f32 ? 16 : 8)) == 0, "%s: dy must be %d-byte aligned", who, dy_f32 ? 16 : 8);
+    DCLIP_REQUIRE((uintptr_t)x % 16 == 0 && (uintptr_t)dx_acc % 16 == 0 && (uintptr_t)gamma % 16 == 0, "%s: x, dx_acc and gamma must be 16-byte aligned", who);
+    DCLIP_REQUIRE((uintptr_t)dx_bf16 % 8 == 0, "%s: dx_bf16 must be 8-byte aligned", who);
+    const int nv = (int)((D + 255) / 256);
+    int blocks = (int)((M + 7) / 8);
+    if (blocks > 256) blocks = 256;
+    TraceScope tr(DCLIP_TRACE_LN_BWD, 12.0 * (double)M * D, (double)M * D * ((dy_f32 ? 4.0 : 2.0) + (seed ? 8.0 : 12.0) + (dx_bf16 ? 2.0 : 0.0)), stream, (int)M, (int)D, 0, 0);
+    hipStream_t st = (hipStream_t)stream;
+#define LN_BWD_GO(F32, SEEDED) hipLaunchKernelGGL((ln_bwd_kernel<NV, F32, SEEDED>), dim3(blocks), dim3(512), (size_t)3 * 8 * NV * 256 * 4, st, dy, lddy, x, ldx, row_index, gamma, mean, rstd, dx_acc, lddx, (bf16_t*)dx_bf16, lddb, dgamma, dbeta, colsum_acc, (int)M, (int)D, seed, seed_pick, (int)seed_n)
+    LN_DISPATCH(nv,
+        if (seed) { if (dy_f32) LN_BWD_GO(true, true); else LN_BWD_GO(false, true); }
+        else { if (dy_f32) LN_BWD_GO(true, false); else LN_BWD_GO(false, false); });
+#undef LN_BWD_GO
+    return dclip_check_launch(who);
+}
+
 extern "C" int dclip_layernorm_bwd(const void* dy, int64_t lddy, int dy_f32, const float* x, int64_t ldx,
                                    const int32_t* row_index, const float* gamma, const float* mean, const float* rstd,
                                    float* dx_acc, int64_t lddx, void* dx_bf16, int64_t lddb, float* dgamma, float* dbeta,
                                    float* colsum_acc, int64_t M, int64_t D, void* stream) {
-    DCLIP_REQUIRE(dy && x && gamma && mean && rstd && dx_acc, "dclip_layernorm_bwd: null operand");
-    DCLIP_REQUIRE(M > 0, "dclip_layernorm_bwd: need M > 0 (M=%ld)", (long)M);
-    DCLIP_REQUIRE(D > 0 && D % 4 == 0 && D <= 1024, "dclip_layernorm_bwd: need 0 < D <= 1024, D %% 4 == 0 (D=%ld)", (long)D);
-    DCLIP_REQUIRE(lddy % 4 == 0 && ldx % 4 == 0 && lddx % 4 == 0 && (!dx_bf16 || lddb % 4 == 0),
-                  "dclip_layernorm_bwd: row strides must be multiples of 4 (lddy=%ld, ldx=%ld, lddx=%ld, lddb=%ld)", (long)lddy, (long)ldx, (long)lddx, (long)lddb);
-    DCLIP_REQUIRE(((uintptr_t)dy % (dy_f32 ? 16 : 8)) == 0, "dclip_layernorm_bwd: dy must be %d-byte aligned", dy_f32 ? 16 : 8);
-    DCLIP_REQUIRE((uintptr_t)x % 16 == 0 && (uintptr_t)dx_acc % 16 == 0 && (uintptr_t)gamma % 16 == 0, "dclip_layernorm_bwd: x, dx_acc and gamma must be 16-byte aligned");
-    DCLIP_REQUIRE((uintptr_t)dx_bf16 % 8 == 0, "dclip_layernorm_bwd: dx_bf16 must be 8-byte aligned");
-    const int nv = (int)((D + 255) / 256);
-    int blocks = (int)((M + 7) / 8);
-    if (blocks > 256) blocks = 256;
-    TraceScope tr(DCLIP_TRACE_LN_BWD, 12.0 * (double)M * D, (double)M * D * ((dy_f32 ? 4.0 : 2.0) + 12.0 + (dx_bf16 ? 2.0 : 0.0)), stream, (int)M, (int)D, 0, 0);
-    hipStream_t st = (hipStream_t)stream;
-    LN_DISPATCH(nv,
-        if (dy_f32) hipLaunchKernelGGL((ln_bwd_kernel<NV, true>), dim3(blocks), dim3(512), (size_t)3 * 8 * NV * 256 * 4, st, dy, lddy, x, ldx, row_index, gamma, mean, rstd, dx_acc, lddx, (bf16_t*)dx_bf16, lddb, dgamma, dbeta, colsum_acc, (int)M, (int)D);
-        else hipLaunchKernelGGL((ln_bwd_kernel<NV, false>), dim3(blocks), dim3(512), (size_t)3 * 8 * NV * 256 * 4, st, dy, lddy, x, ldx, row_index, gamma, mean, rstd, dx_acc, lddx, (bf16_t*)dx_bf16, lddb, dgamma, dbeta, colsum_acc, (int)M, (int)D));
-    return dclip_check_launch("dclip_layernorm_bwd");
-}
+    return ln_bwd_launch(dy, lddy, dy_f32, x, ldx, row_index, gamma, mean, rstd, dx_acc, lddx, dx_bf16, lddb, dgamma, dbeta, colsum_acc, M, D,
+                         nullptr, nullptr, 1, stream, "dclip_layernorm_bwd");
+}
+
+extern "C" int dclip_layernorm_bwd_seeded(const void* dy, int64_t lddy, int dy_f32, const float* x, int64_t ldx, const float* gamma,
+                                          const float* mean, const float* rstd, const float* seed, const int32_t* pick, int64_t B,
+                                          int64_t N, float* dx_acc, int64_t lddx, void* dx_bf16, int64_t lddb, float* dgamma,
+                                          float* dbeta, float* colsum_acc, int64_t D, void* stream) {
+    DCLIP_REQUIRE(seed && pick && B > 0 && N > 0 && B * N < (1LL << 31), "dclip_layernorm_bwd_seeded: bad seed argument");
+    DCLIP_REQUIRE((uintptr_t)seed % 16 == 0, "dclip_layernorm_bwd_seeded: seed must be 16-byte aligned");
+    DCLIP_REQUIRE(seed != dx_acc, "dclip_layernorm_bwd_seeded: seed and dx_acc must not alias");
+    return ln_bwd_launch(dy, lddy, dy_f32, x, ldx, nullptr, gamma, mean, rstd, dx_acc, lddx, dx_bf16, lddb, dgamma, dbeta, colsum_acc, B * N, D,
+                         seed, pick, N, stream, "dclip_layernorm_bwd_seeded");
+}
diff --git a/distillclip_amd/ops.py b/distillclip_amd/ops.py
--- a/distillclip_amd/ops.py
+++ b/distillclip_amd/ops.py
@@ -68,6 +68,18 @@
     return dw
 
 
+def gemm_tn_acc_colsum(a, b, dw, db, splits=4, tile256=False, workspace=True):
+    _chk(a, b, dw, db)
+    assert a.dtype == torch.bfloat16 and b.dtype == torch.bfloat16 and dw.dtype == torch.float32 and db.dtype == torch.float32
+    M, P = a.shape
+    Q = b.shape[1]
+    assert b.shape[0] == M and tuple(dw.shape) == (P, Q) and dw.stride(1) == 1 and tuple(db.shape) == (P,) and db.stride(0) == 1
+    ws = _tn_workspace(a.device) if workspace else None
+    lib().dclip_gemm_tn_acc_colsum(_p(a), a.stride(0), _p(b), b.stride(0), _p(dw), dw.stride(0), _p(db), M, P, Q, splits, 1 if tile256 else 0,
+                                   _p(ws), 0 if ws is None else ws.numel(), _stream())
+    return dw, db
+
+
 def colsum_acc(x, db):
     _chk(x, db)
     assert x.dtype == torch.bfloat16 and db.dtype == torch.float32
@@ -94,6 +106,16 @@
     lib().dclip_layernorm_bwd(_p(dy), dy.stride(0), 1 if dy.dtype == torch.float32 else 0, _p(x), x.stride(0),
                               _p(row_index), _p(gamma), _p(mean), _p(rstd), _p(dx_acc), dx_acc.stride(0), _p(dx_bf16),
                               dx_bf16.stride(0) if dx_bf16 is not None else 0, _p(dgamma), _p(dbeta), _p(colsum), M, D, _stream())
+
+
+def layernorm_bwd_seeded(dy, x, gamma, mean, rstd, seed, pick, N, dx_acc, *, dx_bf16=None, dgamma=None, dbeta=None, colsum=None):
+    _chk(dy, x, gamma, mean, rstd, seed, pick, dx_acc, dx_bf16, dgamma, dbeta)
+    M, D = dy.shape
+    B = pick.numel()
+    assert M == B * N and tuple(seed.shape) == (B, D) and seed.is_contiguous() and pick.dtype == torch.int32
+    lib().dclip_layernorm_bwd_seeded(_p(dy), dy.stride(0), 1 if dy.dtype == torch.float32 else 0, _p(x), x.stride(0), _p(gamma), _p(mean),
+                                     _p(rstd), _p(seed), _p(pick), B, N, _p(dx_acc), dx_acc.stride(0), _p(dx_bf16),
+                                     dx_bf16.stride(0) if dx_bf16 is not None else 0, _p(dgamma), _p(dbeta), _p(colsum), D, _stream())
 
 
 def attn_nt(a, lda, bm, ldb, B, H, N, hd, alpha=1.0, out_dtype=torch.float32):
diff --git a/include/dclip.h b/include/dclip.h
--- a/include/dclip.h
+++ b/include/dclip.h
@@ -35,6 +35,8 @@
 int64_t dclip_gemm_tn_atomic_fallbacks(void);
 int dclip_gemm_tn_acc(const void* A, int64_t lda, const void* B, int64_t ldb, float* dW, int64_t ldo,
                       int64_t M, int64_t P, int64_t Q, int splits, void* workspace, size_t ws_bytes, void* stream);
+int dclip_gemm_tn_acc_colsum(const void* A, int64_t lda, const void* B, int64_t ldb, float* dW, int64_t ldo, float* dA_colsum,
+                             int64_t M, int64_t P, int64_t Q, int splits, int tile256, void* workspace, size_t ws_bytes, void* stream);
 
 int dclip_colsum_acc(const void* X, int64_t ld, float* db, int64_t M, int64_t N, void* stream);
 
@@ -48,6 +50,10 @@
                         const float* gamma, const float* mean, const float* rstd, float* dx_acc, int64_t lddx,
                         void* dx_bf16, int64_t lddb, float* dgamma, float* dbeta, float* colsum_acc, int64_t M, int64_t D,
                         void* stream);
+int dclip_layernorm_bwd_seeded(const void* dy, int64_t lddy, int dy_f32, const float* x, int64_t ldx, const float* gamma,
+                               const float* mean, const float* rstd, const float* seed, const int32_t* pick, int64_t B, int64_t N,
+                               float* dx_acc, int64_t lddx, void* dx_bf16, int64_t lddb, float* dgamma, float* dbeta,
+                               float* colsum_acc, int64_t D, void* stream);
 
 int dclip_attn_nt(const void* A, int64_t lda, const void* Bm, int64_t ldb, void* C, int out_f32, int64_t B, int64_t H,
                   int64_t N, int64_t Np, int64_t hd, float alpha, void* stream);
```

After: 18770 pairs/s (median of 6 runs). Within noise of the previous version (+0.5%).
